# SysCV/LiDAR_snow_sim

Hardware: AMD Instinct MI355X
Metric: augmented points/s/GPU (64x2048 sweep, 2.5 mm/h); HBM roofline % -- value: rows resident in HBM when the clock starts (device-resident API: augment_batch on CUDA tensors); with H2D of the rows and D2H of the results inside the clock: value_pcie_inclusive (higher is better)
Workload: dtype f64

## Files before the change

### lidar_snow_sim_amd/csrc/sg_common.h

```cpp
#pragma once
#include <stddef.h>
#include <stdint.h>

#define SG_PI 3.141592653589793
#define SG_TWO_PI (2 * SG_PI)
#define SG_RBINS 1230
#define SG_NBINS 2048
#define SG_BIN_MARGIN 1e-6
#define SG_BEAM_MARGIN 1e-9
#define SG_TBL_STRIDE 16
#define SG_BLKREC 8
#define SG_HITS_UNDECIDED 0x40000000
#define SG_MAX_LASERS 256
#define SG_LCAP 63
#define SG_TILE 1024

struct SgEntry {
    double phi;
    double x, y, r;
    double t0, t1;
    double rho;
    uint32_t flags;
    uint32_t src;
};

#define SG_OV_CAP 16
#define SG_OV_STRIDE (2 + 3 * SG_OV_CAP)
#ifndef SG_QSTEPS
#define SG_QSTEPS 16
#define SG_QSTEP_M 8.0
#endif

struct SgTable {
    const SgEntry *entries;
    const uint32_t *bin_start;
    const uint32_t *bin_q;
    uint32_t n_bins;
    uint32_t n_entries;
    double inv_bin_w;
    uint32_t n_flakes;
    uint32_t max_bin;
    const uint32_t *bin_qs;
    uint32_t qs_steps;
    float qs_per_m;
};

struct SgLasers {
    double focal_slope[SG_MAX_LASERS];
    double focal_offset[SG_MAX_LASERS];
    int32_t min_i[SG_MAX_LASERS];
    int32_t max_i[SG_MAX_LASERS];
    int32_t n;
};

#define SG_REC_LABEL_SHIFT 8
#define SG_REC_COPY (1u << 10)
#define SG_REC_HAS_I (1u << 11)
#define SG_REC_SLOT (1u << 31)
#define SG_REC_K_SHIFT 12
#define SG_MAX_CLASSES 4

#if defined(__HIPCC__) || defined(__HIP__)
typedef int2 int2_t;
#else
struct int2_t { int32_t x, y; };
#endif

struct SgBeamArgs {
    const void *rows;
    const int64_t *frame_off;
    int32_t n_frames;
    int64_t n_total;
    int64_t uniform_rows;
    float inv_uniform_rows;
    const int32_t *perm;
    const void *srows;
    const int32_t *frame_unsorted;
    const SgTable *frame_tables;
    const SgLasers *las;
    const double *rgrid;
    double beam_div_deg;
    uint32_t *rec;
    uint32_t *rec_q;
    void *rng;
    int32_t *status;
    int32_t *tier_hint;
    unsigned long long *diff2;
    int32_t exact_math;
    int32_t n_cls;
    int32_t cls_cap[SG_MAX_CLASSES];
    const int32_t *seg_blk;
    const int64_t *seg_start;
    const int32_t *seg_cnt;
    const int32_t *seg_frame;
    const int32_t *seg_n;
    const int32_t *seg_of_blk;
    int64_t grid_blocks;
    int32_t q_chunk;
    int64_t blk_lo, blk_hi;
    const int32_t *chunk_blk;
    int32_t chunk;
    uint32_t *dq;
    int32_t *dq_g;
    uint16_t *dq_sc;
    unsigned long long *qn;
    int2_t *pw_items;
    int32_t *pw_count;
    int2_t *pw_items1;
    int32_t front_max;
    int64_t n_regions_ub;
    int32_t blk_rows;
    int32_t kp_lds_quarters;
    int64_t dq_n;
    int32_t *tier_list;
    int32_t *tier_info;
    int64_t tier_stride;
    int32_t *tier_sparse;
    int32_t *tn, *tbase;
    int32_t cls;
    int32_t work_lo, work_hi;
    int32_t work_hint;
    int32_t *redo_list;
    int32_t *redo_cnt;
    double *tq;
    uint16_t *tq_sc;
    int32_t tq_cap;
    double *ov;
    uint16_t *ov_sc;
    int32_t ov_cap;
    int32_t ov_list;
    double *h_lists;
    int32_t h_cap, h_lanes;
    int32_t *dbg_count;
    double *dbg_rj;
    double *dbg_ratio;
    int32_t dbg_cap;
};

struct SgFov {
    int32_t enabled;
    int32_t reserved_;
    double m[12];
    double p[12];
    double img_h, img_w;
};

#ifdef __cplusplus
extern "C" {
#endif
int sg_launch_expand_rows(const void *xyzi, const uint8_t *ch, void *rows, int64_t n, void *stream);
int sg_launch_sort(const void *rows, int dtype, const int64_t *frame_off, int n_frames, int64_t n_total,
                   int32_t *tile_hist, int32_t *tile_base, uint16_t *rank, uint8_t *ch8, int32_t *perm, int32_t *status,
                   int64_t max_tiles_per_frame, const double *lean_plane, double *lean_part, int32_t *tile_unsorted,
                   int32_t *frame_unsorted, void *srows, int identity_perm ,
                   int phase , void *stream);
int sg_launch_gather_rows(const void *rows, int dtype, const int64_t *frame_off, int n_frames, int64_t n_total, int64_t max_frame,
                          const int32_t *perm, void *srows, int32_t *frame_unsorted, int32_t *status, void *stream);
int sg_launch_beams(const SgBeamArgs *args, int dtype, int lmax, int direct, void *stream);
int sg_launch_power(const SgBeamArgs *args, int dtype, int lmax, void *stream, int plan_only ,
                    void *ev_few , int which );
int sg_launch_tier_gather(const SgBeamArgs *args, void *stream);
int sg_launch_power_list(const SgBeamArgs *args, int dtype, int lmax, void *stream);
int sg_launch_huge(const SgBeamArgs *args, int dtype, void *stream);
int sg_launch_tier_scan(const SgBeamArgs *args, int dtype, int lmax, void *stream);
int sg_launch_rows(const SgBeamArgs *args, int dtype, int lmax, void *stream);
int sg_launch_segments(const int64_t *frame_off, int n_frames, const int32_t *tile_base, int64_t max_tiles, const int32_t *table_ids,
                       int n_las, int n_tables, int block, unsigned long long *tbl_cnt, unsigned long long *tbl_base, int32_t *seg_blk,
                       int64_t *seg_start, int32_t *seg_cnt, int32_t *seg_frame, int32_t *seg_n, int32_t *seg_of_blk,
                       int32_t *chunk_blk, const SgTable *tables, SgTable *resolved , void *stream);
int sg_launch_segments_small(const int64_t *frame_off, int n_frames, const int32_t *tile_base, int64_t max_tiles, const int32_t *table_ids,
                             int n_las, int n_tables, int block, int32_t *seg_blk, int64_t *seg_start, int32_t *seg_cnt, int32_t *seg_frame,
                             int32_t *seg_n, int32_t *seg_of_blk, int32_t *chunk_blk, const SgTable *tables, SgTable *resolved,
                             unsigned long long *zero, int64_t n_zero, void *stream);
int sg_beams_block(int lmax);
int sg_launch_resolve_tables(const SgTable *tables, int n_tables, const int32_t *table_ids, int64_t n, SgTable *out, void *stream);
struct SgPackOut {
    uint32_t *meta;
    void *inten;
    void *mv;
    int64_t *mv_counts;
    int32_t *tile_mv, *tile_mv_base;
};
int sg_launch_compact(const void *rows, const void *srows, const int32_t *frame_unsorted, int dtype, const uint32_t *rec, const uint32_t *rec_q, const void *rng, const double *thr_poly, uint8_t *keep, const int32_t *perm,
                      const int64_t *frame_off, int n_frames, int64_t n_total, int32_t *tile_cnt,
                      int32_t *tile_base, void *out_rows, int32_t *out_src, int64_t *out_counts,
                      int64_t *out_stats, const unsigned long long *diff2, const SgFov *fov, int64_t max_tiles_per_frame,
                      const SgPackOut *pack , unsigned long long *tiles_done , void *stream);
int sg_launch_finish_aligned(const void *rows, const void *srows, const int32_t *frame_unsorted, int dtype, const uint32_t *rec, const uint32_t *rec_q, const void *rng,
                             const double *thr_poly, const int32_t *perm, const int64_t *frame_off, int n_frames, int32_t *tile_cnt, int32_t *tile_base,
                             void *out_rows, uint8_t *out_keep, int64_t *out_counts, int64_t *out_stats, const unsigned long long *diff2, const SgFov *fov,
                             int64_t max_tiles_per_frame, unsigned long long *tiles_done , void *stream);
int sg_launch_crop_count(const void *rows, int dtype, const int64_t *frame_off, int n_frames, uint8_t *keep, int32_t *tile_cnt,
                         int32_t *tile_base, int64_t *out_counts, int64_t *stats_scratch, const SgFov *fov, int64_t max_tiles, void *stream);
int sg_launch_crop_scatter(const void *rows, int dtype, const uint8_t *keep, const double *gate , const int64_t *frame_off, const int64_t *new_off,
                           int n_frames, const int32_t *tile_base, void *out_rows, int32_t *crop_src, int64_t max_tiles, void *stream);
int sg_launch_mask_front(const void *rows, int dtype, const uint8_t *keep_in, const double *weather, const int64_t *frame_off, int n_frames, void *out_rows ,
                         uint8_t *out_keep, int32_t *tile_cnt, int32_t *tile_base, int64_t *counts, int64_t *new_off, void *crows, int32_t *map,
                         int64_t max_tiles, void *stream);
int sg_launch_finish_aligned_masked(const void *crows, const void *srows, const int32_t *frame_unsorted, int dtype, const uint32_t *rec, const uint32_t *rec_q,
                                    const void *rng, const double *thr_poly, const int32_t *perm, const int64_t *c_off, const int64_t *in_off,
                                    const int32_t *map, int n_frames, int32_t *tile_cnt, int32_t *tile_base, void *out_rows, uint8_t *out_keep,
                                    int64_t *out_counts, int64_t *out_stats, const unsigned long long *diff2, const SgFov *fov, int64_t max_tiles_per_frame,
                                    unsigned long long *tiles_done , void *stream);
int sg_launch_fov_mask(const void *rows, int dtype, int64_t n, const uint8_t *keep_in, uint8_t *out_keep, const SgFov *fov, void *stream);
struct SgDrorGrid;
int sg_launch_dror(const void *rows, int dtype, int64_t n, const int64_t *frame_off, int n_frames, const uint8_t *keep_in, const struct SgDrorGrid *g,
                   uint32_t *entry, uint32_t *cell_of, void *sorted, uint8_t *out_keep, int32_t *out_nb, void *stream);
struct SgVoxelGrid;
int sg_launch_voxelize(const void *rows, int dtype, int64_t n, const int64_t *frame_off, int n_frames, const uint8_t *keep_in, const struct SgVoxelGrid *g,
                       unsigned long long *table, uint32_t *slot_of, uint8_t *first, uint32_t *order, int32_t *tile_cnt, int32_t *tile_base, int32_t *fbase,
                       int32_t *m, uint32_t *span, void *out_voxels, int32_t *out_coords, int32_t *out_num_points, int32_t *out_voxel_offsets,
                       int32_t *out_voxel_of, void *stream);
struct SgFpsRange;
int sg_launch_fps(const void *rows, int dtype, int64_t n, const int64_t *frame_off, int n_frames, const uint8_t *keep_in, const struct SgFpsRange *range,
                  int32_t n_samples, int32_t n_features, void *sx, void *sy, void *sz, void *st, int32_t *ssrc, int32_t *out_index, void *out_points,
                  void *out_dist, int32_t *out_usable, void *stream);
int sg_launch_fps_sectors(const void *rows, int dtype, int64_t n, int64_t max_frame, const int64_t *frame_off, int n_frames, const uint8_t *keep_in,
                          const struct SgFpsRange *range, int32_t n_samples, int32_t n_features, int32_t n_sectors, const void *rois, int32_t n_rois,
                          int32_t roi_features, double roi_margin, void *sx, void *sy, void *sz, void *st, int32_t *ssrc, int8_t *sec, void *rec,
                          int32_t *tile, int32_t *seg, int32_t *out_index, void *out_points, void *out_dist, int32_t *out_usable,
                          int32_t *out_offsets, int32_t *out_count, int8_t *out_sector_of, double *out_reach2, void *stream);
struct SgBallGrid;
int sg_launch_ball(const void *rows, int dtype, int64_t n, const int64_t *frame_off, int n_frames, const uint8_t *keep_in, const struct SgFpsRange *range,
                   const struct SgBallGrid *g, int32_t n_centres, const void *centres, int32_t centre_features, int n_radii, const double *radii,
                   const int *n_samples, int32_t n_features, uint32_t *entry, uint32_t *cell_of, void *sx, void *sy, void *sz, int32_t *ssrc,
                   int32_t *out_index, int32_t *out_count, void *out_points, void *stream);
struct SgRangeGeom;
int sg_launch_range(const void *rows, int dtype, int64_t n, const int64_t *frame_off, int n_frames, const uint8_t *keep_in, const int32_t *ring,
                    const struct SgRangeGeom *g, int32_t n_features, unsigned long long *key, void *out_image, int32_t *out_index,
                    int32_t *out_pixel_of, int32_t *out_count, void *stream);
struct SgNnGrid;
int sg_launch_nn(const void *rows, int dtype, int64_t n, const int64_t *frame_off, int n_frames, const uint8_t *keep_in, const struct SgFpsRange *range,
                 const struct SgNnGrid *g, int32_t n_centres, const void *centres, int32_t centre_features, int k, uint32_t *entry, int32_t *box, void *rec,
                 int32_t *out_index, void *out_dist, void *out_weight, void *stream);
struct SgBoxRec;
int sg_launch_box(const void *rows, int dtype, int64_t n, const int64_t *frame_off, int n_frames, const uint8_t *keep_in, int32_t n_boxes,
                  const void *boxes, int32_t box_features, const double *pose_in, struct SgBoxRec *rec, unsigned long long *table, int32_t *out_box_of,
                  int32_t *out_count, void *out_local, double *out_pose, void *stream);
int sg_launch_roipool(const void *rows, int dtype, int64_t n, int64_t max_frame, const int64_t *frame_off, int n_frames, const uint8_t *keep_in,
                      int32_t n_rois, const void *rois, int32_t roi_features, const double *ew, int32_t n_samples, int32_t num_features,
                      const double *pose_in, struct SgBoxRec *rec, unsigned long long *table, int32_t *run_cnt, int32_t *out_index, int32_t *out_count,
                      void *out_points, void *out_local, double *out_pose, void *stream);
int sg_launch_roi_members(const void *rows, int dtype, int64_t n, int64_t max_frame, const int64_t *frame_off, int n_frames, const uint8_t *keep_in,
                          int32_t n_rois, const void *rois, int32_t roi_features, const double *ew, int32_t n_slots, const double *pose_in,
                          struct SgBoxRec *rec, unsigned long long *table, int32_t *run_cnt, int32_t *out_index, int32_t *out_count, double *out_pose,
                          void *stream);
int sg_launch_roiaware(const void *rows, int dtype, int64_t n, int64_t max_frame, const int64_t *frame_off, int n_frames, const uint8_t *keep_in,
                       int32_t n_rois, const void *rois, int32_t roi_features, const double *ew, const int32_t *grid, int32_t max_points, int32_t cap,
                       const float *features, int32_t channels, const double *pose_in, struct SgBoxRec *rec, unsigned long long *table, int32_t *run_cnt,
                       int32_t *list, int32_t *sorted, int32_t *offset, int32_t *out_roi_count, int32_t *out_count, int32_t *out_index, float *out_max,
                       int32_t *out_argmax, float *out_avg, double *out_pose, void *stream);
int sg_launch_iou(int n_frames, int32_t M, const void *boxes_a, int32_t a_features, int32_t B, const void *boxes_b, int32_t b_features, int dtype, int mode,
                  const double *pose_a, const double *pose_b, double *rec, void *out_iou, int32_t *out_best, void *out_best_iou, void *stream);
int sg_launch_nms(int n_frames, int32_t B, const void *boxes, int32_t box_features, const void *scores, int dtype, int mode, double iou_thresh,
                  double score_thresh, int32_t post_max, const double *pose_in, double *rec, int32_t *order, int32_t *n_cand, int32_t *out_index,
                  int32_t *out_count, void *out_boxes, void *out_scores, uint8_t *out_kept, void *stream);
struct SgTargetCfg;
int sg_launch_sample_rois(const struct SgTargetCfg *cfg, int n_frames, int32_t n_rois, const void *rois, int32_t roi_features, const void *overlap,
                          const int32_t *assign, int32_t n_gt, const void *gt, int32_t gt_features, int dtype, uint64_t seed, const uint64_t *d_step,
                          const double *pose_in, int32_t *out_index, void *out_rois, void *out_roi_iou, int32_t *out_gt_index, void *out_gt_of_rois,
                          uint8_t *out_reg_valid, void *out_cls_label, int32_t *out_segments, int32_t *out_class_count, double *out_pose,
                          void *out_gt_local, void *stream);
struct SgAnchorCfg;
int sg_launch_assign_anchors(const struct SgAnchorCfg *cfg, int n_frames, int32_t n_anchors, const void *anchors, int32_t anchor_features,
                             const int32_t *anchor_class, int32_t n_gt, const void *gt, int32_t gt_features, int dtype, void *recs,
                             unsigned long long *top, int32_t *blk, int32_t *out_label, int32_t *out_gt_index, int32_t *out_count,
                             int32_t *out_gt_count, void *out_iou, void *stream);
struct SgCenterCfg;
int sg_launch_assign_centers(const struct SgCenterCfg *cfg, int n_frames, int32_t n_gt, const void *gt, int32_t gt_features, int dtype, void *recs,
                             float *out_heatmap, int32_t *out_gt_index, int32_t *out_ind, uint8_t *out_mask, void *out_offset, int32_t *out_radius,
                             int32_t *out_count, uint8_t *out_state, void *stream);
struct SgPasteGroups;
struct SgPasteFrame;
int sg_launch_paste(const void *rows, int dtype, int64_t n_total, int64_t max_frame, const int64_t *off, int n_frames, const uint8_t *keep, int32_t n_gt,
                    const void *gt, int32_t gt_features, const double *pose_in, const void *bank_points, const int64_t *bank_off, const void *bank_boxes,
                    const double *bank_pose, const int32_t *class_off, const struct SgPasteGroups *groups, const double *ew, uint64_t seed,
                    const uint64_t *d_step, int32_t *table, struct SgPasteFrame *frames, unsigned long long *grid, void *out_rows, uint8_t *out_keep, void *out_gt, int32_t *out_object,
                    int32_t *out_state, int32_t *out_source, int32_t *out_count, double *out_pose, void *stream);
struct SgSceneCfg;
int sg_launch_scene(const void *rows, int dtype, int64_t n_total, int64_t max_frame, const int64_t *off, int n_frames, const uint8_t *keep, int32_t B,
                    const void *gt, int32_t Cb, const double *pose_in, const struct SgSceneCfg *cfg, uint64_t seed, const uint64_t *d_step, const int32_t *box_of,
                    struct SgBoxRec *box_rec, unsigned long long *box_table, int32_t *box_of_own, double *tries, double *rowrec, void *out_rows, uint8_t *out_keep,
                    void *out_gt, double *out_world, int32_t *out_state, int32_t *out_tried, double *out_local, double *out_pose, double *out_tries,
                    void *stream);
#ifdef __cplusplus
}
#endif
```

### lidar_snow_sim_amd/csrc/sg_host.h

```cpp
#pragma once
#include <hip/hip_runtime.h>

#include <algorithm>
#include <array>
#include <cmath>
#include <cstdio>
#include <cstdlib>
#include <cstring>
#include <string>
#include <vector>

#include "../../include/snowgpu.h"
#include "sg_common.h"
#include "sg_prepass.h"
#include "sg_plane.h"
#include "sg_assemble.h"
#include "sg_device_args.h"

#pragma GCC visibility push(hidden)

struct DeviceTable {
    SgEntry *entries = nullptr;
    uint32_t *bin_start = nullptr;
    uint32_t *bin_q = nullptr;
    uint32_t *bin_qs = nullptr;
    SgTable desc{};
};

template <typename T> struct DevBuf {
    T *p = nullptr;
    size_t cap = 0;
    int ensure(size_t n)
    {
        if (n <= cap) return 0;
        if (p) (void)hipFree(p);
        p = nullptr;
        cap = 0;
        size_t want = n + n / 4 + 64;
        hipError_t e = hipMalloc((void **)&p, want * sizeof(T));
        if (e != hipSuccess) return (int)e;
        cap = want;
        return 0;
    }
    void release() { if (p) (void)hipFree(p); p = nullptr; cap = 0; }
};

struct __attribute__((visibility("default"))) snowgpu_ctx {
    int device = 0;
    hipStream_t stream = nullptr;
    hipStream_t aux = nullptr;
    hipStream_t aux2 = nullptr;
    hipStream_t aux3 = nullptr;
    int32_t *tier_hint_h = nullptr, *tier_hint_d = nullptr;
    hipEvent_t ev_fork0 = nullptr, ev_join0 = nullptr;
    hipEvent_t ev_fork = nullptr, ev_join = nullptr;
    hipEvent_t ev_fp = nullptr, ev_join2 = nullptr;
    hipEvent_t ev_few = nullptr;
    hipEvent_t ev_lists = nullptr, ev_join3 = nullptr;
    std::string err;
    std::vector<DeviceTable> tables;
    SgTable *d_tables = nullptr;
    size_t d_tables_cap = 0;
    bool tables_dirty = true;
    uint32_t max_flakes = 0;
    SgLasers h_las{};
    SgLasers *d_las = nullptr;
    double *d_rgrid = nullptr;
    int32_t *d_status = nullptr;
    SgFov fov{};
    int fov_pre = 0;
    DevBuf<uint8_t> rows_crop;
    DevBuf<int32_t> crop_src, crop_out_src;
    DevBuf<int64_t> crop_counts, crop_off, crop_stats;
    DevBuf<uint32_t> dror_entry, dror_cell;
    DevBuf<uint8_t> dror_sorted;
    DevBuf<unsigned long long> vox_table;
    DevBuf<uint32_t> vox_slot, vox_order, vox_span;
    DevBuf<uint8_t> vox_first;
    DevBuf<int32_t> vox_tile_cnt, vox_tile_base, vox_fbase, vox_m;
    DevBuf<uint8_t> fps_x, fps_y, fps_z, fps_t;
    DevBuf<int32_t> fps_src;
    DevBuf<int8_t> fpss_sec;
    DevBuf<double> fpss_roi;
    DevBuf<int32_t> fpss_tile, fpss_seg;
    DevBuf<uint32_t> ball_entry, ball_cell;
    DevBuf<uint8_t> ball_x, ball_y, ball_z;
    DevBuf<int32_t> ball_src;
    DevBuf<unsigned long long> range_key;
    DevBuf<uint32_t> nn_entry;
    DevBuf<int32_t> nn_box;
    DevBuf<uint8_t> nn_rec;
    DevBuf<double> box_rec;
    DevBuf<unsigned long long> box_table;
    DevBuf<double> roi_rec;
    DevBuf<unsigned long long> roi_table;
    DevBuf<int32_t> roi_runs;
    DevBuf<double> rv_rec;
    DevBuf<unsigned long long> rv_table;
    DevBuf<int32_t> rv_runs, rv_list, rv_sorted, rv_offset;
    DevBuf<double> iou_rec;
    DevBuf<int32_t> nms_order, nms_cand;
    DevBuf<double> anchor_rec;
    DevBuf<unsigned long long> anchor_top;
    DevBuf<int32_t> anchor_blk;
    DevBuf<double> center_rec;
    DevBuf<int32_t> paste_runs;
    DevBuf<uint8_t> paste_frames;
    DevBuf<unsigned long long> paste_grid;
    DevBuf<double> scene_rowrec, scene_tries, scene_box_rec;
    DevBuf<unsigned long long> scene_box_table;
    DevBuf<int32_t> scene_box_of;
    DevBuf<int32_t> tile_hist, tile_base, perm, ctile_cnt, ctile_base, table_ids, out_src;
    DevBuf<uint8_t> srows;
    DevBuf<int32_t> tile_unsorted, frame_unsorted;
    DevBuf<unsigned long long> seg_tbl_cnt, seg_tbl_base;
    DevBuf<int32_t> seg_blk, seg_cnt, seg_frame, seg_n, seg_of_blk;
    DevBuf<int64_t> seg_start;
    DevBuf<uint32_t> rec, rec_q;
    DevBuf<uint8_t> rng;
    DevBuf<uint32_t> dq;
    DevBuf<int32_t> dq_g;
    DevBuf<uint16_t> dq_sc;
    DevBuf<unsigned long long> qn;
    DevBuf<int2_t> pw_items;
    DevBuf<double> ov;
    DevBuf<uint16_t> ov_sc;
    DevBuf<int32_t> tier_list, tier_sparse, tbase, redo_list;
    DevBuf<double> tq[SG_MAX_CLASSES];
    DevBuf<uint16_t> tq_sc[SG_MAX_CLASSES];
    DevBuf<double> h_lists;
    int64_t tier_cap_override = 0;
    int first_tier_override = 0;
    int few = 2;
    int heavy_tail = -1;
    int tier_rows = -1;
    hipStream_t lane_stream[3] = {nullptr, nullptr, nullptr};
    int stats_early = -1;
    int prepass_with_few = -1;
    bool serial = false;
    DevBuf<int32_t> chunk_blk;
    DevBuf<uint16_t> rank;
    DevBuf<uint8_t> keep, rows_in, rows_out;
    DevBuf<int64_t> frame_off, out_counts, out_stats;
    DevBuf<double> thr_poly, plane, dbg_rj, dbg_ratio, user_thr, out_thr;
    DevBuf<int32_t> user_perm;
    DevBuf<int32_t> dbg_count;
    DevBuf<SgTable> frame_tables;
    SgPrepassScratch prepass{};
    SgPlaneScratch plane_scr{};
    SgPlaneParams plane_par{SG_PLANE_REFERENCE, 1024, 5, 0, -1.55};
    DevBuf<double> plane_est, wet_plane_est;
    DevBuf<int32_t> plane_info;
    int64_t resident_rows = -1;
    int resident_dtype = -1;
    std::vector<int64_t> resident_off;
    DevBuf<int32_t> stats_hist;
    DevBuf<double> stats_rec;
    DevBuf<uint8_t> snow_rows;
    DevBuf<int32_t> snow_src, wet_flags;
    DevBuf<int64_t> snow_counts, wet_counts;
    DevBuf<double> wet_rows, wet_plane;
    std::vector<hipEvent_t> ev_start, ev_stop;
    int ev_used = 0;
    bool prof = false;
    hipStream_t prof_stream = nullptr;
    int exact_math = 0;
    snowgpu_ctx *root = nullptr;
    std::vector<snowgpu_ctx *> lanes;
    int pipe_lanes = 2;
    char *mail_up_h = nullptr, *mail_dn_h = nullptr;
    size_t mail_up_cap = 0, mail_dn_cap = 0;
    DevBuf<uint8_t> mail_up_d, mail_dn_d;
    hipStream_t s_h2d = nullptr, s_d2h = nullptr;
    std::vector<hipEvent_t> pipe_ev;
    DevBuf<int64_t> pipe_off;
    DevBuf<int32_t> pipe_status;
    int64_t pipe_rows = (int64_t)3 << 19;
    std::vector<double> wet_lines;
    DevBuf<double> d_wet_lines;
    int wet_estimation = 0;
    uint64_t wet_seed = 0;
    DevBuf<double> wet_fit;
    int wet_fit_frames = 0;
    int32_t h_status[8] = {0, -1, 0, 0, 0, 0, 0, 0};
    int result_mode = 0;
    int asm_threads = 0;
    DevBuf<uint32_t> pk_meta;
    DevBuf<uint8_t> pk_int, pk_mv;
    DevBuf<int64_t> pk_mvcnt;
    DevBuf<int32_t> pk_tile_mv, pk_tile_mv_base;
    char *st_pk = nullptr;
    size_t st_pk_cap = 0;
    std::vector<hipEvent_t> pk_ev;
    AsmPool *pool = nullptr;
    double pk_times[4] = {0, 0, 0, 0};
    const uint8_t *in_channels = nullptr;
    DevBuf<uint8_t> rows_c4, rows_ch;
    snowgpu_threshold_fn thr_fn = nullptr;
    void *thr_user = nullptr;
    char *thr_stage = nullptr;
    size_t thr_stage_cap = 0;
    std::vector<hipEvent_t> thr_ev;
};

#define HIPCHK(ctx, call)                                                                         \
    do {                                                                                          \
        hipError_t e__ = (call);                                                                  \
        if (e__ != hipSuccess) {                                                                  \
            (ctx)->err = std::string(#call) + ": " + hipGetErrorString(e__);                      \
            return SNOWGPU_E_HIP;                                                                 \
        }                                                                                         \
    } while (0)

#define ENSURE(ctx, buf, n)                                                                       \
    do {                                                                                          \
        if ((buf).ensure(n)) { (ctx)->err = "hipMalloc failed for " #buf; return SNOWGPU_E_HIP; } \
    } while (0)

static inline int fail(snowgpu_ctx *ctx, int code, const std::string &msg)
{
    if (ctx) ctx->err = msg;
    return code;
}

static inline std::array<hipEvent_t *, 9> lane_events(snowgpu_ctx *c)
{
    return {&c->ev_fork0, &c->ev_join0, &c->ev_fork, &c->ev_join, &c->ev_join2, &c->ev_lists, &c->ev_join3, &c->ev_few, &c->ev_fp};
}

struct HostCall {
    snowgpu_ctx *ctx;
    bool pipe = false;
    bool drained = false;
    hipError_t drain()
    {
        drained = true;
        hipError_t first = hipSuccess;
        auto sync = [&first](hipStream_t s) { if (s) { hipError_t e = hipStreamSynchronize(s); if (first == hipSuccess) first = e; } };
        if (pipe) {
            if (ctx->pool) ctx->pool->wait_idle();
            sync(ctx->s_h2d);
            for (snowgpu_ctx *ln : ctx->lanes) sync(ln->stream);
        }
        sync(ctx->stream);
        if (pipe) sync(ctx->s_d2h);
        return first;
    }
    ~HostCall() { if (!drained) (void)drain(); }
};

struct BatchDev {
    int n_frames;
    int64_t n_total;
    int64_t max_frame;
    int64_t uniform_rows = 0;
    const int64_t *frame_off;
    const void *rows;
    int dtype;
    const int32_t *table_ids;
    double beam_div_deg;
    const double *thr_poly;
    const double *plane;
    double noise_floor;
    const int32_t *perm;
    void *out_rows;
    int32_t *out_src;
    uint8_t *out_keep = nullptr;
    const int32_t *mask_map = nullptr;
    const int64_t *mask_in_off = nullptr;
    const double *weather = nullptr;
    int64_t *out_counts;
    int64_t *out_stats;
    double *out_thr_poly;
    int32_t *status;
    hipStream_t stream;
    int32_t *dbg_count = nullptr;
    double *dbg_rj = nullptr, *dbg_ratio = nullptr;
    int dbg_cap = 0;
    int32_t *perm_out = nullptr;
    bool no_fov = false;
    bool want_perm = false;
    SgPackOut *pack = nullptr;
    bool serial = false;
    bool defer_thr = false;
};

int run_batch(snowgpu_ctx *ctx, BatchDev &b);
int run_compaction(snowgpu_ctx *ctx, BatchDev &b);
int status_to_error(snowgpu_ctx *ctx, const int32_t st[8]);
int node_of_device(int device);
SgFov make_fov(const double *v2c, const double *r0, const double *p2, int img_h, int img_w);
int wet_settings(snowgpu_ctx *ctx, const SgWetScalars &w, int n_frames, bool take_lines, hipStream_t st, SgWetParams *wp);

#pragma GCC visibility pop

struct SgWeatherDraw;
extern "C" int sg_launch_draw_weather(const SgWeatherDraw *p, int n_frames, uint64_t seed, const uint64_t *d_step, const int32_t *d_set_ids,
                                      int32_t *d_table_ids, double *d_weather, void *stream);
extern "C" int sg_launch_weather_flags(const double *d_weather, int n_frames, int32_t *d_flags, void *stream);

extern "C" int sg_table_index(const SgEntry *entries, const uint32_t *start, uint32_t *q, uint32_t *qs , int qs_steps, double qs_step_m, void *stream);
extern "C" int sg_file_table_stage_a(const double *d_xyr, int64_t k, SgEntry *fl, int32_t *b0, int32_t *span, uint32_t *count,
                                     uint32_t *start, uint32_t *fill, int32_t *misc, void *stream);
extern "C" int sg_file_table_stage_b(int64_t k, const SgEntry *fl, const int32_t *b0, const int32_t *span, const uint32_t *start,
                                     uint32_t *fill, SgEntry *tmp, SgEntry *entries, void *stream);
extern "C" int sg_table_dump(const SgEntry *entries, uint32_t n_entries, double *d_out, void *stream);
extern "C" int sg_sample_table(double occupancy, double scale_mm, double R0, uint64_t seed, int64_t n_cand, double *d_xyr,
                               int64_t cap, int64_t *n_rows, void *stream);
```

### lidar_snow_sim_amd/csrc/snowgpu_api.cpp

```cpp
#include <dlfcn.h>

#include "sg_host.h"
#include "sg_table_host.h"
#include "sg_range_index.h"
#include <cmath>

static void range_grid(double *out)
{
    const double stop = 120 + 299792458.0 * 1e-8;
    const int num = SG_RBINS;
    const double step = stop / (num - 1);
    for (int k = 0; k < num; ++k) {
        double v = (double)k * step + 0.0;
        if (k == num - 1) v = stop;
        out[k] = std::rint(v * 100.0) / 100.0;
    }
}

extern "C" const char *snowgpu_version(void) { return "snowgpu 0.1.0 gfx950 (MI355X) hip"; }

extern "C" int snowgpu_range_grid(double *out)
{
    if (!out) return SNOWGPU_E_INVALID;
    range_grid(out);
    return SNOWGPU_OK;
}

extern "C" const char *snowgpu_last_error(const snowgpu_ctx *ctx) { return ctx ? ctx->err.c_str() : "null context"; }

static int init_streams(snowgpu_ctx *ctx)
{
    HIPCHK(ctx, hipStreamCreateWithFlags(&ctx->stream, hipStreamNonBlocking));
    {
        int least = 0, greatest = 0;
        (void)hipDeviceGetStreamPriorityRange(&least, &greatest);
        HIPCHK(ctx, hipStreamCreateWithPriority(&ctx->aux, hipStreamNonBlocking, 0));
        HIPCHK(ctx, hipStreamCreateWithPriority(&ctx->aux2, hipStreamNonBlocking, greatest));
        HIPCHK(ctx, hipStreamCreateWithPriority(&ctx->aux3, hipStreamNonBlocking, 0));
    }
    for (hipEvent_t *ep : lane_events(ctx)) HIPCHK(ctx, hipEventCreateWithFlags(ep, hipEventDisableTiming));
    if (hipHostMalloc((void **)&ctx->tier_hint_h, 64, hipHostMallocMapped) == hipSuccess) {
        std::memset(ctx->tier_hint_h, 0, 64);
        if (hipHostGetDevicePointer((void **)&ctx->tier_hint_d, ctx->tier_hint_h, 0) != hipSuccess) ctx->tier_hint_d = nullptr;
    } else { (void)hipGetLastError(); ctx->tier_hint_h = nullptr; }
    return SNOWGPU_OK;
}

extern "C" int snowgpu_create(int device, snowgpu_ctx **out)
{
    if (!out) return SNOWGPU_E_INVALID;
    *out = nullptr;
    int n = 0;
    if (hipGetDeviceCount(&n) != hipSuccess || device < 0 || device >= n) return SNOWGPU_E_NO_DEVICE;
    snowgpu_ctx *ctx = new snowgpu_ctx();
    ctx->device = device;
    *out = ctx;
    HIPCHK(ctx, hipSetDevice(device));
    { const char *v = std::getenv("SNOWGPU_TIER_CAP"); ctx->tier_cap_override = v ? std::atoll(v) : 0; }
    { const char *v = std::getenv("SNOWGPU_FIRST_TIER"); ctx->first_tier_override = v ? std::atoi(v) : 0; }
    { const char *v = std::getenv("SNOWGPU_FEW"); ctx->few = v ? std::max(0, std::min(3, std::atoi(v))) : 2; }
    { const char *v = std::getenv("SNOWGPU_HEAVY_TAIL"); ctx->heavy_tail = v ? (v[0] == '1' ? 1 : 0) : -1; }
    { const char *v = std::getenv("SNOWGPU_SERIAL"); ctx->serial = v && v[0] == '1'; }
    { const char *v = std::getenv("SNOWGPU_STATS_EARLY"); ctx->stats_early = v ? (v[0] == '1' ? 1 : 0) : -1; }
    { const char *v = std::getenv("SNOWGPU_PREPASS_WITH_FEW"); ctx->prepass_with_few = v ? (v[0] == '1' ? 1 : 0) : -1; }
    { const char *v = std::getenv("SNOWGPU_TIER_ROWS"); ctx->tier_rows = v ? (v[0] == '1' ? 1 : 0) : -1; }
    if (void *h = dlopen("libc10_hip.so", RTLD_NOLOAD | RTLD_LAZY)) {
        dlclose(h);
        ctx->pipe_lanes = 1;
        ctx->pipe_rows = (int64_t)3 << 20;
    }
    { const char *v = std::getenv("SNOWGPU_PIPE_LANES"); if (v) ctx->pipe_lanes = std::min(std::max(std::atoi(v), 1), 4); }
    int rc = init_streams(ctx);
    if (rc) return rc;
    HIPCHK(ctx, hipMalloc((void **)&ctx->d_las, sizeof(SgLasers)));
    HIPCHK(ctx, hipMalloc((void **)&ctx->d_rgrid, sizeof(double) * SG_RBINS));
    HIPCHK(ctx, hipMalloc((void **)&ctx->d_status, sizeof(int32_t) * 8));
    double grid[SG_RBINS];
    range_grid(grid);
    HIPCHK(ctx, hipMemcpy(ctx->d_rgrid, grid, sizeof(grid), hipMemcpyHostToDevice));
    ctx->h_las.n = 0;
    return SNOWGPU_OK;
}

extern "C" void snowgpu_destroy(snowgpu_ctx *ctx)
{
    if (!ctx) return;
    (void)hipSetDevice(ctx->device);
    for (snowgpu_ctx *ln : ctx->lanes) snowgpu_destroy(ln);
    ctx->lanes.clear();
    if (ctx->stream) (void)hipStreamSynchronize(ctx->stream);
    for (hipStream_t w : {ctx->s_h2d, ctx->s_d2h, ctx->lane_stream[0], ctx->lane_stream[1], ctx->lane_stream[2]}) if (w) { (void)hipStreamSynchronize(w); (void)hipStreamDestroy(w); }
    if (ctx->tier_hint_h) (void)hipHostFree(ctx->tier_hint_h);
    if (ctx->thr_stage) (void)hipHostFree(ctx->thr_stage);
    for (hipEvent_t e : ctx->thr_ev) (void)hipEventDestroy(e);
    if (ctx->mail_up_h) (void)hipHostFree(ctx->mail_up_h);
    if (ctx->mail_dn_h) (void)hipHostFree(ctx->mail_dn_h);
    ctx->mail_up_d.release(); ctx->mail_dn_d.release(); ctx->d_wet_lines.release(); ctx->wet_fit.release();
    delete ctx->pool; ctx->pool = nullptr;
    if (ctx->st_pk) (void)hipHostFree(ctx->st_pk);
    for (hipEvent_t e : ctx->pk_ev) (void)hipEventDestroy(e);
    ctx->pk_meta.release(); ctx->pk_int.release(); ctx->pk_mv.release(); ctx->pk_mvcnt.release(); ctx->pk_tile_mv.release(); ctx->pk_tile_mv_base.release();
    for (hipEvent_t e : ctx->pipe_ev) (void)hipEventDestroy(e);
    ctx->pipe_off.release(); ctx->pipe_status.release();
    for (auto &t : ctx->tables) {
        if (t.entries) (void)hipFree(t.entries);
        if (t.bin_start) (void)hipFree(t.bin_start);
        if (t.bin_q) (void)hipFree(t.bin_q);
        if (t.bin_qs) (void)hipFree(t.bin_qs);
    }
    if (ctx->d_tables) (void)hipFree(ctx->d_tables);
    if (ctx->d_las) (void)hipFree(ctx->d_las);
    if (ctx->d_rgrid) (void)hipFree(ctx->d_rgrid);
    if (ctx->d_status) (void)hipFree(ctx->d_status);
    ctx->tile_hist.release(); ctx->tile_base.release(); ctx->perm.release(); ctx->srows.release(); ctx->tile_unsorted.release(); ctx->frame_unsorted.release();
    ctx->seg_tbl_cnt.release(); ctx->seg_tbl_base.release(); ctx->seg_blk.release(); ctx->seg_cnt.release(); ctx->seg_frame.release();
    ctx->seg_n.release(); ctx->seg_start.release(); ctx->seg_of_blk.release(); ctx->chunk_blk.release();
    ctx->rec.release(); ctx->rec_q.release(); ctx->rng.release(); ctx->dq.release(); ctx->dq_g.release(); ctx->dq_sc.release(); ctx->qn.release(); ctx->pw_items.release(); ctx->ov.release(); ctx->ov_sc.release();
    ctx->redo_list.release(); ctx->rows_c4.release(); ctx->rows_ch.release();
    ctx->tier_list.release(); ctx->tier_sparse.release(); ctx->tbase.release(); ctx->h_lists.release();
    for (int k = 0; k < SG_MAX_CLASSES; ++k) { ctx->tq[k].release(); ctx->tq_sc[k].release(); }
    ctx->ctile_cnt.release(); ctx->ctile_base.release(); ctx->table_ids.release(); ctx->out_src.release();
    ctx->rank.release(); ctx->keep.release(); ctx->rows_in.release(); ctx->rows_out.release();
    ctx->frame_off.release(); ctx->out_counts.release(); ctx->out_stats.release();
    ctx->thr_poly.release(); ctx->plane.release(); ctx->dbg_rj.release(); ctx->dbg_ratio.release();
    ctx->dbg_count.release(); ctx->frame_tables.release(); ctx->user_thr.release(); ctx->out_thr.release(); ctx->user_perm.release();
    ctx->snow_rows.release(); ctx->snow_src.release(); ctx->wet_flags.release(); ctx->snow_counts.release();
    ctx->wet_counts.release(); ctx->wet_rows.release(); ctx->wet_plane.release();
    ctx->rows_crop.release(); ctx->crop_src.release(); ctx->crop_out_src.release(); ctx->crop_counts.release(); ctx->crop_off.release(); ctx->crop_stats.release();
    ctx->dror_entry.release(); ctx->dror_cell.release(); ctx->dror_sorted.release();
    ctx->vox_table.release(); ctx->vox_slot.release(); ctx->vox_order.release(); ctx->vox_span.release(); ctx->vox_first.release();
    ctx->vox_tile_cnt.release(); ctx->vox_tile_base.release(); ctx->vox_fbase.release(); ctx->vox_m.release();
    ctx->fps_x.release(); ctx->fps_y.release(); ctx->fps_z.release(); ctx->fps_t.release(); ctx->fps_src.release();
    ctx->fpss_sec.release(); ctx->fpss_roi.release(); ctx->fpss_tile.release(); ctx->fpss_seg.release();
    ctx->ball_entry.release(); ctx->ball_cell.release(); ctx->ball_x.release(); ctx->ball_y.release(); ctx->ball_z.release(); ctx->ball_src.release();
    ctx->range_key.release();
    ctx->nn_entry.release(); ctx->nn_box.release(); ctx->nn_rec.release();
    ctx->box_rec.release(); ctx->box_table.release();
    ctx->roi_rec.release(); ctx->roi_table.release(); ctx->roi_runs.release();
    ctx->rv_rec.release(); ctx->rv_table.release(); ctx->rv_runs.release(); ctx->rv_list.release(); ctx->rv_sorted.release(); ctx->rv_offset.release();
    ctx->iou_rec.release(); ctx->nms_order.release(); ctx->nms_cand.release();
    ctx->anchor_rec.release(); ctx->anchor_top.release(); ctx->anchor_blk.release();
    ctx->paste_runs.release(); ctx->paste_frames.release(); ctx->paste_grid.release();
    ctx->scene_rowrec.release(); ctx->scene_tries.release(); ctx->scene_box_rec.release(); ctx->scene_box_table.release(); ctx->scene_box_of.release();
    sg_prepass_release(&ctx->prepass);
    sg_plane_release(&ctx->plane_scr);
    ctx->plane_est.release(); ctx->wet_plane_est.release(); ctx->plane_info.release(); ctx->stats_hist.release(); ctx->stats_rec.release();
    for (auto e : ctx->ev_start) (void)hipEventDestroy(e);
    for (auto e : ctx->ev_stop) (void)hipEventDestroy(e);
    for (hipEvent_t *ep : lane_events(ctx)) if (*ep) (void)hipEventDestroy(*ep);
    for (hipStream_t st : {ctx->aux3, ctx->aux2, ctx->aux, ctx->stream})
        if (st) (void)hipStreamDestroy(st);
    delete ctx;
}

extern "C" int snowgpu_set_lasers(snowgpu_ctx *ctx, int n, const double *focal_slope, const double *focal_offset,
                                  const int32_t *min_intensity, const int32_t *max_intensity)
{
    if (!ctx) return SNOWGPU_E_INVALID;
    if (n <= 0 || n > SG_MAX_LASERS || !focal_slope || !focal_offset || !min_intensity || !max_intensity)
        return fail(ctx, SNOWGPU_E_INVALID, "snowgpu_set_lasers: need 1..256 lasers and four arrays");
    HIPCHK(ctx, hipSetDevice(ctx->device));
    for (int i = 0; i < n; ++i) {
        ctx->h_las.focal_slope[i] = focal_slope[i];
        ctx->h_las.focal_offset[i] = focal_offset[i];
        ctx->h_las.min_i[i] = min_intensity[i];
        ctx->h_las.max_i[i] = max_intensity[i];
    }
    ctx->h_las.n = n;
    HIPCHK(ctx, hipMemcpy(ctx->d_las, &ctx->h_las, sizeof(SgLasers), hipMemcpyHostToDevice));
    return SNOWGPU_OK;
}


static int register_table(snowgpu_ctx *ctx, int table_id, SgEntry *entries, uint32_t *bin_start, uint32_t n_entries, uint32_t k,
                          uint32_t max_bin)
{
    if ((size_t)table_id >= ctx->tables.size()) ctx->tables.resize((size_t)table_id + 1);
    DeviceTable &dt = ctx->tables[(size_t)table_id];
    if (dt.entries || dt.bin_start) (void)hipStreamSynchronize(ctx->stream);
    if (dt.entries) (void)hipFree(dt.entries);
    if (dt.bin_start) (void)hipFree(dt.bin_start);
    if (dt.bin_q) (void)hipFree(dt.bin_q);
    if (dt.bin_qs) (void)hipFree(dt.bin_qs);
    dt.entries = entries; dt.bin_start = bin_start; dt.bin_q = nullptr; dt.bin_qs = nullptr;
    dt.desc = SgTable{};
    ctx->tables_dirty = true;
    uint32_t *q = nullptr, *qs = nullptr;
    int e = (int)hipMalloc((void **)&q, (size_t)SG_NBINS * SG_QSTEPS * sizeof(uint32_t));
    static_assert(SG_QS_FILE_STEPS >= 1 && SG_QS_FILE_STEPS <= 64, "k_table_index files one step per lane of a wave");
    static_assert((float)(1.0 / SG_QS_FILE_STEP_M) * SG_QS_FILE_STEP_M == 1.0, "the step length is a power of two");
    if (!e && SG_QS_FITS(max_bin)) e = (int)hipMalloc((void **)&qs, SG_QS_WORDS_OF(SG_QS_FILE_STEPS, SG_NBINS) * sizeof(uint32_t));
    if (!e) e = sg_table_index(entries, bin_start, q, qs, SG_QS_FILE_STEPS, SG_QS_FILE_STEP_M, ctx->stream);
    if (!e) e = (int)hipStreamSynchronize(ctx->stream);
    if (e) {
        if (q) (void)hipFree(q);
        if (qs) (void)hipFree(qs);
        (void)hipFree(entries); (void)hipFree(bin_start);
        dt.entries = nullptr; dt.bin_start = nullptr;
        return fail(ctx, SNOWGPU_E_HIP, std::string("table index: ") + hipGetErrorString((hipError_t)e));
    }
    dt.bin_q = q; dt.bin_qs = qs;
    dt.desc.entries = entries;
    dt.desc.bin_start = bin_start;
    dt.desc.bin_q = q;
    dt.desc.bin_qs = qs;
    dt.desc.qs_steps = qs ? (uint32_t)SG_QS_FILE_STEPS : 0u;
    dt.desc.qs_per_m = (float)(1.0 / SG_QS_FILE_STEP_M);
    dt.desc.n_bins = (uint32_t)SG_NBINS;
    dt.desc.n_entries = n_entries;
    dt.desc.inv_bin_w = SG_NBINS / SG_TWO_PI;
    dt.desc.n_flakes = k;
    dt.desc.max_bin = max_bin;
    ctx->tables_dirty = true;
    ctx->max_flakes = std::max(ctx->max_flakes, k);
    return SNOWGPU_OK;
}

static int file_table_device(snowgpu_ctx *ctx, int table_id, const double *d_xyr, int64_t k)
{
    hipStream_t st = ctx->stream;
    const size_t nb = SG_NBINS;
    DevBuf<SgEntry> fl, tmp;
    DevBuf<int32_t> b0, span, misc;
    DevBuf<uint32_t> count, start, fill;
    auto cleanup = [&]() { fl.release(); tmp.release(); b0.release(); span.release(); misc.release(); count.release(); start.release(); fill.release(); };
    if (fl.ensure((size_t)std::max<int64_t>(k, 1)) || b0.ensure((size_t)std::max<int64_t>(k, 1)) || span.ensure((size_t)std::max<int64_t>(k, 1)) ||
        misc.ensure(2) || count.ensure(nb + 1) || start.ensure(nb + 1) || fill.ensure(nb + 1)) {
        cleanup();
        return fail(ctx, SNOWGPU_E_HIP, "hipMalloc failed while filing a table");
    }
    int e = sg_file_table_stage_a(d_xyr, k, fl.p, b0.p, span.p, count.p, start.p, fill.p, misc.p, st);
    uint32_t n_entries = 0;
    int32_t h_misc[2] = {0, 0};
    if (!e) e = (int)hipMemcpyAsync(&n_entries, start.p + nb, sizeof(uint32_t), hipMemcpyDeviceToHost, st);
    if (!e) e = (int)hipMemcpyAsync(h_misc, misc.p, sizeof h_misc, hipMemcpyDeviceToHost, st);
    if (!e) e = (int)hipStreamSynchronize(st);
    if (e) { cleanup(); return fail(ctx, SNOWGPU_E_HIP, std::string("table filing: ") + hipGetErrorString((hipError_t)e)); }
    if (h_misc[0] > 0) {
        cleanup();
        char buf[128];
        snprintf(buf, sizeof buf, "table row %d is not a disk clear of the origin", 0x7fffffff - h_misc[0]);
        return fail(ctx, SNOWGPU_E_TABLE, buf);
    }
    if ((size_t)n_entries > (size_t)64 * (size_t)std::max<int64_t>(k, 1) + 4096) {
        cleanup();
        return fail(ctx, SNOWGPU_E_TABLE, "flakes so close to the sensor that they cover most azimuths");
    }
    SgEntry *d_entries = nullptr;
    uint32_t *d_start = nullptr;
    if (tmp.ensure((size_t)n_entries + 1) || hipMalloc((void **)&d_entries, ((size_t)n_entries + 1) * sizeof(SgEntry)) != hipSuccess ||
        hipMalloc((void **)&d_start, (nb + 1) * sizeof(uint32_t)) != hipSuccess) {
        if (d_entries) (void)hipFree(d_entries);
        cleanup();
        return fail(ctx, SNOWGPU_E_HIP, "hipMalloc failed while filing a table");
    }
    e = sg_file_table_stage_b(k, fl.p, b0.p, span.p, start.p, fill.p, tmp.p, d_entries, st);
    if (!e) e = (int)hipMemcpyAsync(d_start, start.p, (nb + 1) * sizeof(uint32_t), hipMemcpyDeviceToDevice, st);
    if (!e) e = (int)hipStreamSynchronize(st);
    cleanup();
    if (e) { (void)hipFree(d_entries); (void)hipFree(d_start); return fail(ctx, SNOWGPU_E_HIP, std::string("table filing: ") + hipGetErrorString((hipError_t)e)); }
    return register_table(ctx, table_id, d_entries, d_start, n_entries, (uint32_t)k, (uint32_t)h_misc[1]);
}

extern "C" int snowgpu_file_table_device(snowgpu_ctx *ctx, int table_id, const double *d_xyr, int64_t n_flakes)
{
    if (!ctx) return SNOWGPU_E_INVALID;
    if (table_id < 0 || table_id > (1 << 20) || n_flakes < 0 || (n_flakes > 0 && !d_xyr))
        return fail(ctx, SNOWGPU_E_INVALID, "snowgpu_file_table_device: bad table id or size");
    HIPCHK(ctx, hipSetDevice(ctx->device));
    return file_table_device(ctx, table_id, d_xyr, n_flakes);
}

extern "C" int snowgpu_debug_table(snowgpu_ctx *ctx, int table_id, double *out, int64_t cap_rows)
{
    if (!ctx || !out) return SNOWGPU_E_INVALID;
    if (table_id < 0 || (size_t)table_id >= ctx->tables.size() || !ctx->tables[(size_t)table_id].entries)
        return fail(ctx, SNOWGPU_E_INVALID, "snowgpu_debug_table: unknown table id");
    const DeviceTable &dt = ctx->tables[(size_t)table_id];
    const size_t k = dt.desc.n_flakes;
    if ((int64_t)k > cap_rows) return fail(ctx, SNOWGPU_E_INVALID, "snowgpu_debug_table: buffer too small");
    HIPCHK(ctx, hipSetDevice(ctx->device));
    DevBuf<double> d;
    if (d.ensure(std::max<size_t>(k * 4, 1))) return fail(ctx, SNOWGPU_E_HIP, "hipMalloc failed");
    int e = sg_table_dump(dt.entries, dt.desc.n_entries, d.p, ctx->stream);
    if (!e && k) e = (int)hipMemcpyAsync(out, d.p, sizeof(double) * 4 * k, hipMemcpyDeviceToHost, ctx->stream);
    if (!e) e = (int)hipStreamSynchronize(ctx->stream);
    d.release();
    if (e) return fail(ctx, SNOWGPU_E_HIP, std::string("table dump: ") + hipGetErrorString((hipError_t)e));
    return SNOWGPU_OK;
}

extern "C" int snowgpu_debug_table_bins(snowgpu_ctx *ctx, int table_id, uint32_t *bin_start, int64_t cap_start, void *entries, int64_t cap_entries,
                                        uint32_t *bin_q, int64_t cap_q, uint32_t *bin_qs, int64_t cap_qs, int64_t *info, double *qs_per_m)
{
    if (!ctx || !bin_start || !entries || !bin_q || !bin_qs || !info || !qs_per_m) return SNOWGPU_E_INVALID;
    if (table_id < 0 || (size_t)table_id >= ctx->tables.size() || !ctx->tables[(size_t)table_id].entries)
        return fail(ctx, SNOWGPU_E_INVALID, "snowgpu_debug_table_bins: unknown table id");
    const DeviceTable &dt = ctx->tables[(size_t)table_id];
    const size_t n_start = (size_t)SG_NBINS + 1, n_rec = (size_t)dt.desc.n_entries + 1, n_q = (size_t)SG_NBINS * SG_QSTEPS;
    const size_t n_qs = dt.bin_qs ? SG_QS_WORDS_OF(dt.desc.qs_steps, SG_NBINS) : 0;
    info[0] = dt.desc.n_flakes; info[1] = dt.desc.n_entries; info[2] = dt.desc.max_bin; info[3] = dt.desc.qs_steps; info[4] = dt.bin_qs ? 1 : 0;
    *qs_per_m = (double)dt.desc.qs_per_m;
    if (cap_start < (int64_t)n_start || cap_entries < (int64_t)n_rec || cap_q < (int64_t)n_q || cap_qs < (int64_t)n_qs)
        return fail(ctx, SNOWGPU_E_INVALID, "snowgpu_debug_table_bins: buffer too small (see info)");
    HIPCHK(ctx, hipSetDevice(ctx->device));
    int e = (int)hipMemcpyAsync(bin_start, dt.bin_start, sizeof(uint32_t) * n_start, hipMemcpyDeviceToHost, ctx->stream);
    if (!e) e = (int)hipMemcpyAsync(entries, dt.entries, sizeof(SgEntry) * n_rec, hipMemcpyDeviceToHost, ctx->stream);
    if (!e) e = (int)hipMemcpyAsync(bin_q, dt.bin_q, sizeof(uint32_t) * n_q, hipMemcpyDeviceToHost, ctx->stream);
    if (!e && n_qs) e = (int)hipMemcpyAsync(bin_qs, dt.bin_qs, sizeof(uint32_t) * n_qs, hipMemcpyDeviceToHost, ctx->stream);
    const int es = (int)hipStreamSynchronize(ctx->stream);
    if (!e) e = es;
    if (e) return fail(ctx, SNOWGPU_E_HIP, std::string("table bins: ") + hipGetErrorString((hipError_t)e));
    return SNOWGPU_OK;
}

extern "C" int snowgpu_upload_table(snowgpu_ctx *ctx, int table_id, const double *xyr, int64_t k)
{
    if (!ctx) return SNOWGPU_E_INVALID;
    if (table_id < 0 || table_id > (1 << 20) || k < 0 || (k > 0 && !xyr))
        return fail(ctx, SNOWGPU_E_INVALID, "snowgpu_upload_table: bad table id or size");
    HIPCHK(ctx, hipSetDevice(ctx->device));
    const int nb = SG_NBINS;
    std::vector<SgEntry> entries;
    std::vector<uint32_t> start;
    uint32_t max_bin = 0;
    int64_t bad_row = -1;
    const int frc = sg_file_table_host(xyr, k, entries, start, max_bin, &bad_row);
    if (frc == 1) {
        char buf[160];
        snprintf(buf, sizeof buf, "snowgpu_upload_table: row %lld (%g, %g, %g) is not a disk clear of the origin",
                 (long long)bad_row, xyr[3 * bad_row], xyr[3 * bad_row + 1], xyr[3 * bad_row + 2]);
        return fail(ctx, SNOWGPU_E_TABLE, buf);
    }
    if (frc == 2) return fail(ctx, SNOWGPU_E_TABLE, "snowgpu_upload_table: flakes so close to the sensor that they cover most azimuths");
    const size_t n_entries = start[(size_t)nb];
    SgEntry *d_entries = nullptr;
    uint32_t *d_start = nullptr;
    HIPCHK(ctx, hipMalloc((void **)&d_entries, (n_entries + 1) * sizeof(SgEntry)));
    if (hipMalloc((void **)&d_start, ((size_t)nb + 1) * sizeof(uint32_t)) != hipSuccess) { (void)hipFree(d_entries); return fail(ctx, SNOWGPU_E_HIP, "hipMalloc failed for bin offsets"); }
    HIPCHK(ctx, hipMemcpy(d_entries, entries.data(), (n_entries + 1) * sizeof(SgEntry), hipMemcpyHostToDevice));
    HIPCHK(ctx, hipMemcpy(d_start, start.data(), ((size_t)nb + 1) * sizeof(uint32_t), hipMemcpyHostToDevice));
    return register_table(ctx, table_id, d_entries, d_start, (uint32_t)n_entries, (uint32_t)k, max_bin);
}

extern "C" int snowgpu_free_table(snowgpu_ctx *ctx, int table_id)
{
    if (!ctx) return SNOWGPU_E_INVALID;
    if (table_id < 0 || (size_t)table_id >= ctx->tables.size()) return fail(ctx, SNOWGPU_E_INVALID, "snowgpu_free_table: unknown table id");
    HIPCHK(ctx, hipSetDevice(ctx->device));
    DeviceTable &dt = ctx->tables[(size_t)table_id];
    if (dt.entries || dt.bin_start) HIPCHK(ctx, hipStreamSynchronize(ctx->stream));
    if (dt.entries) { (void)hipFree(dt.entries); dt.entries = nullptr; }
    if (dt.bin_start) { (void)hipFree(dt.bin_start); dt.bin_start = nullptr; }
    if (dt.bin_q) { (void)hipFree(dt.bin_q); dt.bin_q = nullptr; }
    if (dt.bin_qs) { (void)hipFree(dt.bin_qs); dt.bin_qs = nullptr; }
    dt.desc = SgTable{};
    ctx->tables_dirty = true;
    return SNOWGPU_OK;
}

extern "C" int snowgpu_table_count(const snowgpu_ctx *ctx)
{
    if (!ctx) return 0;
    int n = 0;
    for (auto &t : ctx->tables) n += t.entries != nullptr;
    return n;
}

extern "C" int snowgpu_status_error(snowgpu_ctx *ctx, const int32_t *status8)
{
    if (!ctx || !status8) return SNOWGPU_E_INVALID;
    return status_to_error(ctx, status8);
}

extern "C" int snowgpu_sample_table(snowgpu_ctx *ctx, int table_id, double occupancy_ratio, double diameter_scale_mm, double r_0,
                                    uint64_t seed, double *xyr_out, int64_t cap, int64_t *n_out)
{
    if (!ctx) return SNOWGPU_E_INVALID;
    if (!(occupancy_ratio > 0) || !(occupancy_ratio < 0.05) || !(diameter_scale_mm > 0) || !(r_0 > 0.05) || !(r_0 <= 500.0) || !n_out)
        return fail(ctx, SNOWGPU_E_INVALID, "snowgpu_sample_table: need 0 < occupancy < 0.05, scale > 0, 0.05 < R0 <= 500 m");
    HIPCHK(ctx, hipSetDevice(ctx->device));
    const double target = occupancy_ratio * SG_PI * r_0 * r_0;
    const double s_m = diameter_scale_mm / 1000.0;
    const double mean_area = SG_PI * s_m * s_m / 3.0;
    int64_t n_cand = (int64_t)(1.3 * target / mean_area) + 4096;
    int64_t rows = 0;
    DevBuf<double> d_xyr;
    for (int attempt = 0;; ++attempt) {
        if (n_cand > ((int64_t)1 << 27)) return fail(ctx, SNOWGPU_E_INVALID, "snowgpu_sample_table: table would exceed 2^27 candidates");
        if (d_xyr.ensure((size_t)n_cand * 3)) return fail(ctx, SNOWGPU_E_HIP, "hipMalloc failed for the sampled table");
        int rc = sg_sample_table(occupancy_ratio, diameter_scale_mm, r_0, seed, n_cand, d_xyr.p, n_cand, &rows, ctx->stream);
        if (rc == -2 && attempt < 4) { d_xyr.release(); n_cand *= 2; continue; }
        if (rc != 0) {
            d_xyr.release();
            if (rc > 0) return fail(ctx, SNOWGPU_E_HIP, std::string("sampler: ") + hipGetErrorString((hipError_t)rc));
            return fail(ctx, SNOWGPU_E_TABLE, rc == -3 ? "sampler: a dart overlaps more than 4 earlier darts (occupancy too high for this sampler)"
                                                       : "sampler: acceptance did not settle / target area not reached");
        }
        break;
    }
    *n_out = rows;
    int rc = SNOWGPU_OK;
    if (xyr_out) {
        if (cap < rows) rc = fail(ctx, SNOWGPU_E_INVALID, "snowgpu_sample_table: output buffer too small (see *n_out)");
        else if (rows && hipMemcpy(xyr_out, d_xyr.p, sizeof(double) * 3 * (size_t)rows, hipMemcpyDeviceToHost) != hipSuccess)
            rc = fail(ctx, SNOWGPU_E_HIP, "sampler copy failed");
    }
    if (rc == SNOWGPU_OK && table_id >= 0) rc = file_table_device(ctx, table_id, d_xyr.p, rows);
    d_xyr.release();
    return rc;
}

extern "C" int snowgpu_last_status(snowgpu_ctx *ctx, int32_t *out8)
{
    if (!ctx || !out8) return SNOWGPU_E_INVALID;
    std::memcpy(out8, ctx->h_status, sizeof(int32_t) * 8);
    return SNOWGPU_OK;
}

extern "C" int snowgpu_device_numa_node(int device)
{
    int n = 0;
    if (hipGetDeviceCount(&n) != hipSuccess || device < 0 || device >= n) return -1;
    return node_of_device(device);
}

extern "C" int snowgpu_set_result_transfer(snowgpu_ctx *ctx, int mode, int threads)
{
    if (!ctx) return SNOWGPU_E_INVALID;
    if ((mode != 0 && mode != 1) || threads < 0 || threads > 256) return fail(ctx, SNOWGPU_E_INVALID, "snowgpu_set_result_transfer: mode 0 or 1, 0 <= threads <= 256");
    if (mode == 1) {
        if (ctx->pool && threads != ctx->asm_threads) { delete ctx->pool; ctx->pool = nullptr; }
        ctx->asm_threads = threads;
    }
    ctx->result_mode = mode;
    return SNOWGPU_OK;
}

extern "C" int snowgpu_debug_transfer_times(snowgpu_ctx *ctx, double *out4)
{
    if (!ctx || !out4) return SNOWGPU_E_INVALID;
    for (int i = 0; i < 3; ++i) out4[i] = ctx->pk_times[i];
    out4[3] = ctx->pool ? (double)ctx->pool->threads.size() : 0.0;
    return SNOWGPU_OK;
}

extern "C" int snowgpu_set_pipeline(snowgpu_ctx *ctx, int64_t chunk_rows)
{
    if (!ctx || chunk_rows < 0) return SNOWGPU_E_INVALID;
    ctx->pipe_rows = chunk_rows;
    return SNOWGPU_OK;
}

extern "C" int snowgpu_set_wet_lines(snowgpu_ctx *ctx, int n_frames, const double *lines)
{
    if (!ctx) return SNOWGPU_E_INVALID;
    if (n_frames <= 0 || !lines) { ctx->wet_lines.clear(); return SNOWGPU_OK; }
    ctx->wet_lines.assign(lines, lines + (size_t)n_frames * 4);
    return SNOWGPU_OK;
}

extern "C" int snowgpu_set_wet_estimation(snowgpu_ctx *ctx, int method, uint64_t seed)
{
    if (!ctx) return SNOWGPU_E_INVALID;
    if (method != 0 && method != 1) return fail(ctx, SNOWGPU_E_INVALID, "snowgpu_set_wet_estimation: method 0 (linear) or 1 (poly)");
    ctx->wet_estimation = method;
    ctx->wet_seed = seed;
    return SNOWGPU_OK;
}

extern "C" int snowgpu_wet_last_fit(snowgpu_ctx *ctx, int n_frames, double *out)
{
    if (!ctx || !out || n_frames <= 0) return SNOWGPU_E_INVALID;
    if (n_frames != ctx->wet_fit_frames) return fail(ctx, SNOWGPU_E_INVALID, "snowgpu_wet_last_fit: the last wet-ground call had another number of frames");
    HIPCHK(ctx, hipSetDevice(ctx->device));
    HIPCHK(ctx, hipStreamSynchronize(ctx->stream));
    HIPCHK(ctx, hipMemcpy(out, ctx->wet_fit.p, sizeof(double) * 8 * (size_t)n_frames, hipMemcpyDeviceToHost));
    return SNOWGPU_OK;
}

extern "C" int snowgpu_debug_ransac_polyfit(snowgpu_ctx *ctx, int m, const double *x, const double *y, uint64_t seed, uint64_t frame, double *out4)
{
    if (!ctx || !x || !y || !out4) return SNOWGPU_E_INVALID;
    if (m < 3 || m > 50) return fail(ctx, SNOWGPU_E_INVALID, "snowgpu_debug_ransac_polyfit: 3 <= m <= 50");
    HIPCHK(ctx, hipSetDevice(ctx->device));
    DevBuf<double> d;
    if (d.ensure(2 * 50 + 4)) return fail(ctx, SNOWGPU_E_HIP, "hipMalloc failed");
    int rc = SNOWGPU_OK;
    hipStream_t st = ctx->stream;
    hipError_t e = hipMemcpyAsync(d.p, x, sizeof(double) * (size_t)m, hipMemcpyHostToDevice, st);
    if (e == hipSuccess) e = hipMemcpyAsync(d.p + 50, y, sizeof(double) * (size_t)m, hipMemcpyHostToDevice, st);
    if (e == hipSuccess) e = (hipError_t)sg_debug_ransac_quad(d.p, d.p + 50, m, seed, frame, d.p + 100, st);
    if (e == hipSuccess) e = hipMemcpyAsync(out4, d.p + 100, sizeof(double) * 4, hipMemcpyDeviceToHost, st);
    if (e == hipSuccess) e = hipStreamSynchronize(st);
    if (e != hipSuccess) rc = fail(ctx, SNOWGPU_E_HIP, std::string("ransac tap: ") + hipGetErrorString(e));
    d.release();
    return rc;
}

extern "C" int snowgpu_set_exact_math(snowgpu_ctx *ctx, int on)
{
    if (!ctx) return SNOWGPU_E_INVALID;
    ctx->exact_math = on ? 1 : 0;
    return SNOWGPU_OK;
}

extern "C" int snowgpu_set_serial(snowgpu_ctx *ctx, int on)
{
    if (!ctx) return SNOWGPU_E_INVALID;
    ctx->serial = on != 0;
    return SNOWGPU_OK;
}

extern "C" int snowgpu_lane_stream(snowgpu_ctx *ctx, int level, void **stream)
{
    if (!ctx || !stream || level < 0 || level > 2) return SNOWGPU_E_INVALID;
    *stream = nullptr;
    HIPCHK(ctx, hipSetDevice(ctx->device));
    if (!ctx->lane_stream[level]) {
        int least = 0, greatest = 0;
        (void)hipDeviceGetStreamPriorityRange(&least, &greatest);
        const int prio = level == 0 ? greatest : level == 2 ? least : (least + greatest) / 2;
        HIPCHK(ctx, hipStreamCreateWithPriority(&ctx->lane_stream[level], hipStreamNonBlocking, prio));
    }
    *stream = (void *)ctx->lane_stream[level];
    return SNOWGPU_OK;
}

extern "C" int snowgpu_host_alloc(snowgpu_ctx *ctx, size_t bytes, void **ptr)
{
    if (!ctx || !ptr) return SNOWGPU_E_INVALID;
    *ptr = nullptr;
    HIPCHK(ctx, hipSetDevice(ctx->device));
    HIPCHK(ctx, hipHostMalloc(ptr, std::max<size_t>(bytes, 8), hipHostMallocPortable));
    return SNOWGPU_OK;
}

extern "C" int snowgpu_host_free(snowgpu_ctx *ctx, void *ptr)
{
    (void)ctx;
    if (!ptr) return SNOWGPU_OK;
    return hipHostFree(ptr) == hipSuccess ? SNOWGPU_OK : SNOWGPU_E_HIP;
}

extern "C" int snowgpu_profile_begin(snowgpu_ctx *ctx, int max_launches)
{
    if (!ctx || max_launches <= 0) return SNOWGPU_E_INVALID;
    HIPCHK(ctx, hipSetDevice(ctx->device));
    while ((int)ctx->ev_start.size() < max_launches) {
        hipEvent_t a, b;
        HIPCHK(ctx, hipEventCreate(&a));
        HIPCHK(ctx, hipEventCreate(&b));
        ctx->ev_start.push_back(a);
        ctx->ev_stop.push_back(b);
    }
    ctx->ev_used = 0;
    ctx->prof = true;
    return SNOWGPU_OK;
}

extern "C" int snowgpu_profile_end(snowgpu_ctx *ctx, double *beam_kernel_ms, int *n_launches)
{
    if (!ctx || !beam_kernel_ms || !n_launches) return SNOWGPU_E_INVALID;
    HIPCHK(ctx, hipSetDevice(ctx->device));
    ctx->prof = false;
    double sum = 0.0;
    if (ctx->ev_used > 0) HIPCHK(ctx, hipEventSynchronize(ctx->ev_stop[(size_t)ctx->ev_used - 1]));
    for (int i = 0; i < ctx->ev_used; ++i) {
        float ms = 0.f;
        HIPCHK(ctx, hipEventElapsedTime(&ms, ctx->ev_start[(size_t)i], ctx->ev_stop[(size_t)i]));
        sum += ms;
    }
    *beam_kernel_ms = sum;
    *n_launches = ctx->ev_used;
    ctx->ev_used = 0;
    return SNOWGPU_OK;
}

extern "C" int snowgpu_set_fov_precrop(snowgpu_ctx *ctx, int on)
{
    if (!ctx) return SNOWGPU_E_INVALID;
    ctx->fov_pre = on ? 1 : 0;
    return SNOWGPU_OK;
}

SgFov make_fov(const double *v2c, const double *r0, const double *p2, int img_h, int img_w)
{
    SgFov f{};
    f.enabled = 1;
    for (int i = 0; i < 4; ++i)
        for (int j = 0; j < 3; ++j) {
            double acc = 0.0;
            for (int k = 0; k < 3; ++k) acc = acc + v2c[4 * k + i] * r0[3 * j + k];
            f.m[3 * i + j] = acc;
        }
    for (int i = 0; i < 12; ++i) f.p[i] = p2[i];
    f.img_h = img_h; f.img_w = img_w;
    return f;
}

extern "C" int snowgpu_set_fov(snowgpu_ctx *ctx, int enabled, const double *v2c, const double *r0, const double *p2, int img_h, int img_w)
{
    if (!ctx) return SNOWGPU_E_INVALID;
    if (!enabled) { ctx->fov.enabled = 0; return SNOWGPU_OK; }
    if (!v2c || !r0 || !p2 || img_h <= 0 || img_w <= 0) return fail(ctx, SNOWGPU_E_INVALID, "snowgpu_set_fov: need V2C, R0, P2 and an image size");
    ctx->fov = make_fov(v2c, r0, p2, img_h, img_w);
    return SNOWGPU_OK;
}

extern "C" int snowgpu_set_plane_method(snowgpu_ctx *ctx, int method, uint64_t seed, int max_trials, int min_rows, double standard_height)
{
    if (!ctx) return SNOWGPU_E_INVALID;
    if (method < SG_PLANE_REFERENCE || method > SG_PLANE_RANSAC || max_trials < 0 || max_trials > (1 << 16) || min_rows < 0)
        return fail(ctx, SNOWGPU_E_INVALID, "snowgpu_set_plane_method: method 0 (reference), 1 (least squares) or 2 (ransac); 0 <= trials <= 65536");
    ctx->plane_par.method = method;
    ctx->plane_par.seed = seed;
    ctx->plane_par.trials = max_trials > 0 ? max_trials : 1024;
    ctx->plane_par.min_rows = min_rows;
    ctx->plane_par.std_height = standard_height;
    return SNOWGPU_OK;
}

extern "C" int snowgpu_set_threshold_callback(snowgpu_ctx *ctx, snowgpu_threshold_fn fn, void *user)
{
    if (!ctx) return SNOWGPU_E_INVALID;
    ctx->thr_fn = fn; ctx->thr_user = fn ? user : nullptr;
    return SNOWGPU_OK;
}
```

### lidar_snow_sim_amd/csrc/snowgpu_batch.cpp

```cpp
#include "sg_host.h"
#include "sg_launch.h"
#include "sg_queue.h"

static int sync_tables(snowgpu_ctx *ctx)
{
    if (!ctx->tables_dirty) return SNOWGPU_OK;
    const size_t n = std::max<size_t>(ctx->tables.size(), 1);
    if (n > ctx->d_tables_cap) {
        if (ctx->d_tables) { (void)hipStreamSynchronize(ctx->stream); (void)hipFree(ctx->d_tables); }
        HIPCHK(ctx, hipMalloc((void **)&ctx->d_tables, n * sizeof(SgTable)));
        ctx->d_tables_cap = n;
    }
    std::vector<SgTable> h(n);
    for (size_t i = 0; i < ctx->tables.size(); ++i) h[i] = ctx->tables[i].desc;
    HIPCHK(ctx, hipMemcpy(ctx->d_tables, h.data(), n * sizeof(SgTable), hipMemcpyHostToDevice));
    ctx->tables_dirty = false;
    return SNOWGPU_OK;
}

static void choose_tiers(const snowgpu_ctx *ctx, double beam_div_deg, int tiers[4], int *n_tiers)
{
    const double expect = (double)ctx->max_flakes * (beam_div_deg * (SG_PI / 180.0)) / SG_TWO_PI;
    int first = expect <= 24.0 ? 4 : (expect <= 48.0 ? 8 : (expect <= 96.0 ? 16 : SG_LCAP));
    if (ctx->first_tier_override == 4 || ctx->first_tier_override == 8 || ctx->first_tier_override == 16 ||
        ctx->first_tier_override == SG_LCAP)
        first = ctx->first_tier_override;
    int n = 0;
    for (int c : {4, 8, 16, SG_LCAP})
        if (c >= first) tiers[n++] = c;
    *n_tiers = n;
}

static int64_t tier_queue_cap(const snowgpu_ctx *ctx, int lmax, int64_t n)
{
    if (ctx->tier_cap_override > 0) return std::min<int64_t>(ctx->tier_cap_override, std::max<int64_t>(n, 1));
    const int64_t slot_bytes = (int64_t)sizeof(double) * (3 * (int64_t)lmax + 2) + 2;
    if (std::max<int64_t>(n, 1) * slot_bytes <= ((int64_t)1 << 30)) return std::max<int64_t>(n, 1);
    const int64_t div = lmax <= 8 ? 4 : (lmax <= 16 ? 16 : 64);
    return std::min<int64_t>(std::max<int64_t>(n, 1), std::max<int64_t>(n / div, 4096));
}

static int launch_compaction(snowgpu_ctx *ctx, BatchDev &b, const int32_t *perm, const double *thr, size_t regions, int64_t max_tiles);

int run_batch(snowgpu_ctx *ctx, BatchDev &b)
{
    snowgpu_ctx *R = ctx->root ? ctx->root : ctx;
    if (R->h_las.n <= 0) return fail(ctx, SNOWGPU_E_INVALID, "snowgpu_set_lasers has not been called");
    if (b.beam_div_deg <= 0 || b.beam_div_deg >= 45.0)
        return fail(ctx, SNOWGPU_E_INVALID, "beam divergence must be in (0, 45) degrees");
    int rc = sync_tables(R);
    if (rc) { if (R != ctx) ctx->err = R->err; return rc; }
    const int64_t max_tiles = sg_tiles(b.max_frame);
    const size_t n = (size_t)b.n_total;
    const size_t esz = b.dtype == 0 ? 4 : 8;
    hipStream_t st = b.stream;
    const bool serial = R->serial || b.serial;
    hipStream_t s_aux = serial ? st : ctx->aux, s_aux2 = serial ? st : ctx->aux2, s_aux3 = serial ? st : ctx->aux3;
    HIPCHK(ctx, hipMemsetAsync(b.status, 0, sizeof(int32_t) * 8, st));
    if (n == 0) {
        HIPCHK(ctx, hipMemsetAsync(b.status + 1, 0xff, sizeof(int32_t), st));
        HIPCHK(ctx, hipMemsetAsync(b.out_counts, 0, sizeof(int64_t) * (size_t)b.n_frames, st));
        HIPCHK(ctx, hipMemsetAsync(b.out_stats, 0, sizeof(int64_t) * 3 * (size_t)b.n_frames, st));
        if (b.pack) HIPCHK(ctx, hipMemsetAsync(b.pack->mv_counts, 0, sizeof(int64_t) * (size_t)b.n_frames, st));
        return SNOWGPU_OK;
    }
    const double *thr = b.thr_poly;
    bool pre_forked = false;
    const bool fuse_stats = !b.thr_poly && !b.defer_thr && !b.perm && (b.plane != nullptr || R->plane_par.method == SG_PLANE_REFERENCE);
    const double *early_plane = b.plane;
    double *lean_part = nullptr;
    if (fuse_stats) {
        if (!early_plane) {
            ENSURE(ctx, ctx->plane_est, (size_t)b.n_frames * 4);
            ENSURE(ctx, ctx->plane_info, (size_t)b.n_frames * 4);
            int pe = sg_plane_run(&ctx->plane_scr, &R->plane_par, b.rows, b.dtype, b.frame_off, nullptr, b.n_frames, b.n_total, b.max_frame,
                                  ctx->plane_est.p, ctx->plane_info.p, st);
            if (pe) return fail(ctx, SNOWGPU_E_HIP, std::string("plane estimate: ") + (pe > 0 ? hipGetErrorString((hipError_t)pe) : "allocation"));
            early_plane = ctx->plane_est.p;
        }
        lean_part = sg_prepass_reserve_tiles(&ctx->prepass, b.n_frames, b.max_frame);
        if (!lean_part) return fail(ctx, SNOWGPU_E_HIP, "prepass: allocation");
    }
    bool hist_early = false;
    const bool stats_early = fuse_stats && !serial && early_plane == b.plane && (R->stats_early < 0 ? b.n_frames > 16 : R->stats_early == 1);
    auto launch_prepass = [&]() -> int {
        HIPCHK(ctx, hipEventRecord(ctx->ev_fork0, st));
        HIPCHK(ctx, hipStreamWaitEvent(s_aux2, ctx->ev_fork0, 0));
        const double *pl = fuse_stats ? early_plane : b.plane;
        if (!pl) {
            ENSURE(ctx, ctx->plane_est, (size_t)b.n_frames * 4);
            ENSURE(ctx, ctx->plane_info, (size_t)b.n_frames * 4);
            int pe = sg_plane_run(&ctx->plane_scr, &R->plane_par, b.rows, b.dtype, b.frame_off, nullptr, b.n_frames, b.n_total, b.max_frame,
                                  ctx->plane_est.p, ctx->plane_info.p, s_aux2);
            if (pe) return fail(ctx, SNOWGPU_E_HIP, std::string("plane estimate: ") + (pe > 0 ? hipGetErrorString((hipError_t)pe) : "allocation"));
            pl = ctx->plane_est.p;
        }
        int e = sg_prepass_run(&ctx->prepass, b.rows, b.dtype, b.frame_off, b.n_frames, b.n_total, b.max_frame, pl,
                               b.noise_floor, ctx->thr_poly.p, b.status, s_aux2, fuse_stats ? 1 : 0, ctx->srows.p, ctx->frame_unsorted.p, hist_early ? 1 : 0, b.weather);
        if (e) return fail(ctx, SNOWGPU_E_HIP, std::string("prepass: ") + (e > 0 ? hipGetErrorString((hipError_t)e) : "allocation"));
        if (b.out_thr_poly)
            HIPCHK(ctx, hipMemcpyAsync(b.out_thr_poly, ctx->thr_poly.p, sizeof(double) * 3 * (size_t)b.n_frames, hipMemcpyDeviceToDevice, s_aux2));
        HIPCHK(ctx, hipEventRecord(ctx->ev_join0, s_aux2));
        pre_forked = true;
        return SNOWGPU_OK;
    };
    if (!thr && b.defer_thr) {
    } else if (!thr) {
        ENSURE(ctx, ctx->thr_poly, (size_t)b.n_frames * 3);
        thr = ctx->thr_poly.p;
        if (!serial) {
            HIPCHK(ctx, hipEventRecord(ctx->ev_fork0, st));
            HIPCHK(ctx, hipStreamWaitEvent(s_aux2, ctx->ev_fork0, 0));
            int he = sg_prepass_clear_hist(&ctx->prepass, b.n_frames, s_aux2);
            if (he) return fail(ctx, SNOWGPU_E_HIP, std::string("prepass: ") + (he > 0 ? hipGetErrorString((hipError_t)he) : "allocation"));
            hist_early = true;
            if (fuse_stats && stats_early) {
                int se = sg_prepass_stats_early(&ctx->prepass, b.rows, b.dtype, b.frame_off, b.n_frames, b.max_frame, early_plane, s_aux2);
                if (se) return fail(ctx, SNOWGPU_E_HIP, std::string("prepass statistics: ") + (se > 0 ? hipGetErrorString((hipError_t)se) : "allocation"));
            }
        }
    } else if (b.out_thr_poly) {
        HIPCHK(ctx, hipMemcpyAsync(b.out_thr_poly, thr, sizeof(double) * 3 * (size_t)b.n_frames, hipMemcpyDeviceToDevice, st));
    }
    const int32_t *perm = b.perm;
    ENSURE(ctx, ctx->srows, n * 5 * esz);
    ENSURE(ctx, ctx->frame_unsorted, (size_t)b.n_frames);
    if (!perm) {
        ENSURE(ctx, ctx->tile_hist, (size_t)b.n_frames * (size_t)max_tiles * 256);
        ENSURE(ctx, ctx->tile_base, (size_t)b.n_frames * (size_t)max_tiles * 256);
        ENSURE(ctx, ctx->tile_unsorted, (size_t)b.n_frames * (size_t)max_tiles);
        ENSURE(ctx, ctx->rank, n);
        ENSURE(ctx, ctx->perm, n);
        ENSURE(ctx, ctx->keep, n);
        int e = sg_launch_sort(b.rows, b.dtype, b.frame_off, b.n_frames, b.n_total, ctx->tile_hist.p, ctx->tile_base.p,
                               ctx->rank.p, ctx->keep.p, ctx->perm.p, b.status, max_tiles, (fuse_stats && !stats_early) ? early_plane : nullptr, (fuse_stats && !stats_early) ? lean_part : nullptr,
                               ctx->tile_unsorted.p, ctx->frame_unsorted.p, ctx->srows.p, b.want_perm ? 1 : 0, 1, st);
        if (e) return fail(ctx, SNOWGPU_E_HIP, std::string("sort launch: ") + hipGetErrorString((hipError_t)e));
        perm = ctx->perm.p;
    } else {
        int e = sg_launch_gather_rows(b.rows, b.dtype, b.frame_off, b.n_frames, b.n_total, b.max_frame, perm, ctx->srows.p, ctx->frame_unsorted.p, b.status, st);
        if (e) return fail(ctx, SNOWGPU_E_HIP, std::string("gather launch: ") + hipGetErrorString((hipError_t)e));
    }
    b.perm_out = const_cast<int32_t *>(perm);
    const int64_t n_ft = (int64_t)b.n_frames * R->h_las.n;
    ENSURE(ctx, ctx->frame_tables, (size_t)n_ft);
    int tiers[4], n_tiers = 0;
    choose_tiers(R, b.beam_div_deg, tiers, &n_tiers);
    const int first_block = sg_beams_block(tiers[0]);
    const bool use_seg = !b.perm && R->tables.size() <= 65536 && b.n_frames <= (1 << 22)
                         && b.n_total < ((int64_t)1 << 31);
    if (b.mask_map && !use_seg) return fail(ctx, SNOWGPU_E_INVALID, "a masked batch needs the segment order of the pass over all rows: at most 65536 tables and 2^22 frames");
    if (use_seg) {
        const size_t P = (size_t)b.n_frames * 256;
        ENSURE(ctx, ctx->seg_tbl_cnt, (R->tables.size() + 1) * SG_TBL_STRIDE); ENSURE(ctx, ctx->seg_tbl_base, R->tables.size() + 1);
        ENSURE(ctx, ctx->seg_blk, P); ENSURE(ctx, ctx->seg_cnt, P);
        ENSURE(ctx, ctx->seg_frame, P); ENSURE(ctx, ctx->seg_start, P); ENSURE(ctx, ctx->seg_n, 2);
        ENSURE(ctx, ctx->seg_of_blk, ((size_t)((b.n_total + first_block - 1) / first_block) + P) * SG_BLKREC);
        ENSURE(ctx, ctx->chunk_blk, 2);
    }
    const int64_t total_blocks_ub = (b.n_total + first_block - 1) / first_block + (use_seg ? (int64_t)b.n_frames * 256 : 0);
    static_assert(SG_MAX_CLASSES * sizeof(int32_t) == 2 * sizeof(unsigned long long), "a region's tier counters are two 64-bit words");
    const size_t q_chunk = 8 * (size_t)first_block;
    const size_t regions = std::max<size_t>((size_t)b.n_frames * 256, n / q_chunk + 2);
    const size_t zero_words = 3 * regions + 2 * (size_t)b.n_frames + 8;
    ENSURE(ctx, ctx->qn, zero_words);
    ENSURE(ctx, ctx->tbase, SG_MAX_CLASSES * regions);
    bool seg_small = false;
    if (use_seg) {
        const int se = sg_launch_segments_small(b.frame_off, b.n_frames, ctx->tile_base.p, max_tiles, b.table_ids, R->h_las.n, (int)R->tables.size(), first_block,
                                                ctx->seg_blk.p, ctx->seg_start.p, ctx->seg_cnt.p, ctx->seg_frame.p, ctx->seg_n.p, ctx->seg_of_blk.p,
                                                ctx->chunk_blk.p, R->d_tables, ctx->frame_tables.p, ctx->qn.p, (int64_t)zero_words, st);
        if (se > 0) return fail(ctx, SNOWGPU_E_HIP, std::string("segment launch: ") + hipGetErrorString((hipError_t)se));
        seg_small = se == 0;
    }
    if (!seg_small) {
        HIPCHK(ctx, hipEventRecord(ctx->ev_fork, st));
        HIPCHK(ctx, hipStreamWaitEvent(s_aux, ctx->ev_fork, 0));
        int e = 0;
        if (!use_seg) e = sg_launch_resolve_tables(R->d_tables, (int)R->tables.size(), b.table_ids, n_ft, ctx->frame_tables.p, s_aux);
        if (e) return fail(ctx, SNOWGPU_E_HIP, std::string("table resolve launch: ") + hipGetErrorString((hipError_t)e));
        if (use_seg) {
            e = sg_launch_segments(b.frame_off, b.n_frames, ctx->tile_base.p, max_tiles, b.table_ids, R->h_las.n, (int)R->tables.size(), first_block,
                                   ctx->seg_tbl_cnt.p, ctx->seg_tbl_base.p, ctx->seg_blk.p, ctx->seg_start.p, ctx->seg_cnt.p, ctx->seg_frame.p,
                                   ctx->seg_n.p, ctx->seg_of_blk.p, ctx->chunk_blk.p, R->d_tables, ctx->frame_tables.p, s_aux);
            if (e) return fail(ctx, SNOWGPU_E_HIP, std::string("segment launch: ") + hipGetErrorString((hipError_t)e));
        }
        HIPCHK(ctx, hipEventRecord(ctx->ev_join, s_aux));
    }
    if (!b.perm) {
        int e = sg_launch_sort(b.rows, b.dtype, b.frame_off, b.n_frames, b.n_total, ctx->tile_hist.p, ctx->tile_base.p,
                               ctx->rank.p, ctx->keep.p, ctx->perm.p, b.status, max_tiles, nullptr, nullptr,
                               ctx->tile_unsorted.p, ctx->frame_unsorted.p, ctx->srows.p, b.want_perm ? 1 : 0, 2, st);
        if (e) return fail(ctx, SNOWGPU_E_HIP, std::string("sort launch: ") + hipGetErrorString((hipError_t)e));
    }
    ENSURE(ctx, ctx->rec, n);
    ENSURE(ctx, ctx->rec_q, n);
    ENSURE(ctx, ctx->rng, n * esz);
    ENSURE(ctx, ctx->keep, n);
    ENSURE(ctx, ctx->tier_list, n * (size_t)n_tiers);
    ENSURE(ctx, ctx->tier_sparse, n * (size_t)n_tiers);
    ENSURE(ctx, ctx->ctile_cnt, (size_t)b.n_frames * (size_t)max_tiles + 1);
    ENSURE(ctx, ctx->ctile_base, (size_t)b.n_frames * (size_t)max_tiles + 1);
    SgBeamArgs a{};
    a.rows = b.rows; a.frame_off = b.frame_off; a.n_frames = b.n_frames; a.n_total = b.n_total; a.perm = perm;
    a.srows = ctx->srows.p; a.frame_unsorted = ctx->frame_unsorted.p;
    a.uniform_rows = (b.uniform_rows > 0 && b.n_total < ((int64_t)1 << 31)) ? b.uniform_rows : 0;
    a.inv_uniform_rows = a.uniform_rows > 0 ? 1.0f / (float)a.uniform_rows : 0.0f;
    a.las = R->d_las; a.frame_tables = ctx->frame_tables.p;
    a.rgrid = R->d_rgrid; a.beam_div_deg = b.beam_div_deg; a.rec = ctx->rec.p; a.rec_q = ctx->rec_q.p;
    a.status = b.status;
    a.rng = ctx->rng.p;
    a.dbg_count = b.dbg_count; a.dbg_rj = b.dbg_rj; a.dbg_ratio = b.dbg_ratio; a.dbg_cap = b.dbg_cap;
    a.exact_math = R->exact_math;
    const int n_cls = n_tiers;
    const bool tier_rows = (R->tier_rows < 0 ? b.n_total <= ((int64_t)1 << 19) : R->tier_rows == 1) && R->tier_cap_override <= 0;
    const int h_lanes = 256;
    const int h_cap = (int)std::min<uint32_t>(std::max<uint32_t>(R->max_flakes, 64u), 8192u);
    a.n_cls = n_cls;
    for (int k = 0; k + 1 < n_cls; ++k) a.cls_cap[k] = tiers[k + 1];
    a.cls_cap[n_cls - 1] = h_cap;
    ENSURE(ctx, ctx->h_lists, (size_t)4 * (size_t)(h_cap + 1) * (size_t)h_lanes);
    a.h_lists = ctx->h_lists.p; a.h_cap = h_cap; a.h_lanes = h_lanes;
    a.tier_list = ctx->tier_list.p; a.tier_stride = b.n_total; a.tier_sparse = ctx->tier_sparse.p;
    if (tier_rows) {
        ENSURE(ctx, ctx->redo_list, n * (size_t)n_tiers);
        a.redo_list = ctx->redo_list.p;
    }
    const bool use_ov = tiers[0] < SG_OV_CAP && n_cls >= 2 && !tier_rows &&
                        R->tier_cap_override <= 0 && n * SG_OV_STRIDE * sizeof(double) <= ((size_t)40 << 30);
    int64_t tq_caps[SG_MAX_CLASSES] = {0, 0, 0, 0};
    for (int k = 0; k + 1 < n_cls && !tier_rows; ++k) {
        if (use_ov && tiers[k + 1] <= SG_OV_CAP) continue;
        tq_caps[k] = tier_queue_cap(R, tiers[k + 1], b.n_total);
        ENSURE(ctx, ctx->tq[k], ((size_t)tq_caps[k] + 64) * (3 * (size_t)tiers[k + 1] + 2));
        ENSURE(ctx, ctx->tq_sc[k], (size_t)tq_caps[k]);
    }
    a.q_chunk = (int32_t)q_chunk;
    {
        const size_t slot_words = (size_t)sg_dq_slot_words(tiers[0], sg_dq_hdr(b.dtype == 0 ? 4 : 8));
        if (n * slot_words * sizeof(uint32_t) > ((size_t)64 << 30))
            return fail(ctx, SNOWGPU_E_INVALID, "batch too large for the dict queue of this table density: split it");
        if (b.n_frames >= (1 << 22)) return fail(ctx, SNOWGPU_E_INVALID, "too many frames in one batch");
        ENSURE(ctx, ctx->dq, (n + 64) * slot_words);
        ENSURE(ctx, ctx->dq_g, n);
        ENSURE(ctx, ctx->dq_sc, n);
        if (!seg_small) HIPCHK(ctx, hipMemsetAsync(ctx->qn.p, 0, sizeof(unsigned long long) * zero_words, st));
        a.tn = (int32_t *)(ctx->qn.p + regions); a.tbase = ctx->tbase.p;
        a.diff2 = ctx->qn.p + 3 * regions;
        int32_t *small = (int32_t *)(ctx->qn.p + 3 * regions + (size_t)b.n_frames);
        a.tier_info = small; a.pw_count = small + 8; a.redo_cnt = small + 12;
        a.dq = ctx->dq.p; a.dq_g = ctx->dq_g.p; a.dq_sc = ctx->dq_sc.p; a.qn = ctx->qn.p; a.dq_n = b.n_total;
        const int lanes = first_block < 64 ? first_block : 64;
        a.n_regions_ub = use_seg ? (int64_t)b.n_frames * 256 : (b.n_total + a.q_chunk - 1) / a.q_chunk;
        a.blk_rows = first_block;
        a.kp_lds_quarters = 2;
        const size_t items_cap = n / (size_t)lanes + 2 * (size_t)a.n_regions_ub + 64;
        ENSURE(ctx, ctx->pw_items, 2 * items_cap);
        a.pw_items = ctx->pw_items.p;
        a.pw_items1 = (R->few > 0 && !b.dbg_count && lanes == 64) ? ctx->pw_items.p + items_cap : nullptr;
        a.front_max = a.pw_items1 ? std::min(R->few, std::min(3, tiers[0])) : 1;
    }
    if (use_ov) {
        ENSURE(ctx, ctx->ov, (n + 256) * SG_OV_STRIDE);
        ENSURE(ctx, ctx->ov_sc, n + 256);
        a.ov = ctx->ov.p; a.ov_sc = ctx->ov_sc.p; a.ov_cap = SG_OV_CAP;
    }
    if (use_seg) {
        a.seg_blk = ctx->seg_blk.p; a.seg_start = ctx->seg_start.p; a.seg_cnt = ctx->seg_cnt.p; a.seg_frame = ctx->seg_frame.p;
        a.seg_n = ctx->seg_n.p; a.seg_of_blk = ctx->seg_of_blk.p; a.chunk_blk = ctx->chunk_blk.p;
    }
    const bool few_first = a.pw_items1 && !serial && b.n_total > ((int64_t)1 << 19);
    bool heavy_tail = false;
    if (few_first && n_cls >= 3 && ctx->tier_hint_d) {
        const volatile int32_t *hint = ctx->tier_hint_h;
        long tail = 0;
        for (int k = 2; k < n_cls && k < SG_MAX_CLASSES; ++k) tail += hint[k];
        heavy_tail = R->heavy_tail < 0 ? (tail >= 4096 && tail * 22 > (long)hint[1]) : R->heavy_tail == 1;
        a.tier_hint = ctx->tier_hint_d;
    }
    if (!seg_small) HIPCHK(ctx, hipStreamWaitEvent(st, ctx->ev_join, 0));
    const bool timed = ctx->prof && ctx->ev_used < (int)ctx->ev_start.size();
    if (timed) { HIPCHK(ctx, hipEventRecord(ctx->ev_start[(size_t)ctx->ev_used], st)); ctx->prof_stream = st; }
    int e = 0;
    {
        const int64_t lin_blocks = (b.n_total + first_block - 1) / first_block;
        if (use_seg) {
            a.chunk = 0;
            a.grid_blocks = total_blocks_ub + b.max_frame / first_block + 2;
        } else {
            a.blk_lo = 0; a.blk_hi = lin_blocks;
            a.grid_blocks = lin_blocks;
        }
        e = sg_launch_beams(&a, b.dtype, tiers[0], 1, st);
        if (!e) e = sg_launch_power(&a, b.dtype, tiers[0], st, 1, nullptr, 3);
        if (!e) {
            HIPCHK(ctx, hipEventRecord(ctx->ev_fp, st));
            HIPCHK(ctx, hipStreamWaitEvent(s_aux, ctx->ev_fp, 0));
            e = sg_launch_power(&a, b.dtype, tiers[0], s_aux, 0, few_first ? ctx->ev_few : nullptr, heavy_tail ? 1 : 3);
        }
        if (!e) {
            const bool pre_with_few = R->prepass_with_few < 0 ? heavy_tail : R->prepass_with_few == 1;
            if (pre_with_few && few_first && !b.thr_poly && !b.defer_thr && !pre_forked) { int prc = launch_prepass(); if (prc) return prc; }
            if (few_first) HIPCHK(ctx, hipStreamWaitEvent(st, ctx->ev_few, 0));
            e = sg_launch_tier_gather(&a, st);
        }
    }
    if (e) return fail(ctx, SNOWGPU_E_HIP, std::string("beam launch: ") + hipGetErrorString((hipError_t)e));
    if (!b.thr_poly && !b.defer_thr && !pre_forked) { int prc = launch_prepass(); if (prc) return prc; }
    const bool side3 = n_cls >= 2;
    const bool tail_main = n_cls >= 3 && !serial && !few_first;
    const bool tail_aux = n_cls >= 3 && !serial && !tail_main;
    if (side3) { HIPCHK(ctx, hipEventRecord(ctx->ev_lists, st)); HIPCHK(ctx, hipStreamWaitEvent(s_aux3, ctx->ev_lists, 0)); }
    if (tail_aux) HIPCHK(ctx, hipStreamWaitEvent(s_aux, ctx->ev_lists, 0));
    if (heavy_tail) {
        e = sg_launch_power(&a, b.dtype, tiers[0], st, 0, nullptr, 2);
    }
    int32_t cls_hint[SG_MAX_CLASSES] = {0, 0, 0, 0};
    if (a.tier_hint && ctx->tier_hint_h) {
        const volatile int32_t *hint = ctx->tier_hint_h;
        const int64_t then_k = hint[SG_MAX_CLASSES];
        if (then_k > 0)
            for (int k = 0; k < SG_MAX_CLASSES; ++k)
                cls_hint[k] = (int32_t)std::min<int64_t>(INT32_MAX / 8, ((int64_t)hint[k] * ((b.n_total >> 10) + 1)) / then_k + 64);
    }
    for (int k = 0; k < n_cls && !e; ++k) {
        a.work_hint = k >= 2 ? cls_hint[k] : 0;
        hipStream_t sk = (k == 0 || (tail_main && k >= 2)) ? st : ((tail_aux && k >= 2) ? s_aux : s_aux3);
        a.seg_blk = nullptr;
        a.cls = k;
        if (k == n_cls - 1) {
            e = sg_launch_huge(&a, b.dtype, sk);
            break;
        }
        const int lmax = tiers[k + 1];
        if (use_ov && lmax <= SG_OV_CAP) {
            a.tq = nullptr; a.tq_sc = nullptr; a.tq_cap = 0; a.ov_list = 1;
            a.work_lo = 0; a.work_hi = (int32_t)std::min<int64_t>(b.n_total, INT32_MAX);
            e = sg_launch_power_list(&a, b.dtype, lmax, sk);
            a.ov_list = 0;
            continue;
        }
        if (tier_rows) {
            a.work_lo = 0; a.work_hi = (int32_t)std::min<int64_t>(b.n_total, INT32_MAX);
            e = sg_launch_rows(&a, b.dtype, lmax, sk);
            continue;
        }
        a.tq = ctx->tq[k].p; a.tq_sc = ctx->tq_sc[k].p; a.tq_cap = (int32_t)tq_caps[k];
        a.work_lo = 0; a.work_hi = (int32_t)tq_caps[k];
        e = sg_launch_tier_scan(&a, b.dtype, lmax, sk);
        if (!e) e = sg_launch_power_list(&a, b.dtype, lmax, sk);
        if (!e && tq_caps[k] < b.n_total) {
            a.work_lo = (int32_t)tq_caps[k]; a.work_hi = (int32_t)std::min<int64_t>(b.n_total, INT32_MAX);
            e = sg_launch_beams(&a, b.dtype, lmax, 0, sk);
        }
    }
    if (e) return fail(ctx, SNOWGPU_E_HIP, std::string("tier launch: ") + hipGetErrorString((hipError_t)e));
    if (side3) { HIPCHK(ctx, hipEventRecord(ctx->ev_join3, s_aux3)); HIPCHK(ctx, hipStreamWaitEvent(st, ctx->ev_join3, 0)); }
    HIPCHK(ctx, hipEventRecord(ctx->ev_join2, s_aux));
    HIPCHK(ctx, hipStreamWaitEvent(st, ctx->ev_join2, 0));
    if (timed) { HIPCHK(ctx, hipEventRecord(ctx->ev_stop[(size_t)ctx->ev_used], st)); ctx->ev_used++; }
    if (pre_forked) HIPCHK(ctx, hipStreamWaitEvent(st, ctx->ev_join0, 0));
    if (b.defer_thr && !b.thr_poly) return SNOWGPU_OK;
    return launch_compaction(ctx, b, perm, thr, regions, max_tiles);
}

static int launch_compaction(snowgpu_ctx *ctx, BatchDev &b, const int32_t *perm, const double *thr, size_t regions, int64_t max_tiles)
{
    snowgpu_ctx *R = ctx->root ? ctx->root : ctx;
    hipStream_t st = b.stream;
    unsigned long long *tiles_done = b.n_total <= ((int64_t)1 << 19) ? ctx->qn.p + 3 * regions + (size_t)b.n_frames + 8 : nullptr;
    if (b.out_keep && b.mask_map) {
        int e = sg_launch_finish_aligned_masked(b.rows, ctx->srows.p, ctx->frame_unsorted.p, b.dtype, ctx->rec.p, ctx->rec_q.p, ctx->rng.p, thr, perm, b.frame_off,
                                                b.mask_in_off, b.mask_map, b.n_frames, ctx->ctile_cnt.p, ctx->ctile_base.p, b.out_rows, b.out_keep, b.out_counts,
                                                b.out_stats, ctx->qn.p + 3 * regions, b.no_fov ? nullptr : &R->fov, max_tiles, tiles_done, st);
        if (e) return fail(ctx, SNOWGPU_E_HIP, std::string("masked aligned finish launch: ") + hipGetErrorString((hipError_t)e));
        return SNOWGPU_OK;
    }
    if (b.out_keep) {
        int e = sg_launch_finish_aligned(b.rows, ctx->srows.p, ctx->frame_unsorted.p, b.dtype, ctx->rec.p, ctx->rec_q.p, ctx->rng.p, thr, perm, b.frame_off, b.n_frames,
                                         ctx->ctile_cnt.p, ctx->ctile_base.p, b.out_rows, b.out_keep, b.out_counts, b.out_stats, ctx->qn.p + 3 * regions,
                                         b.no_fov ? nullptr : &R->fov, max_tiles, tiles_done, st);
        if (e) return fail(ctx, SNOWGPU_E_HIP, std::string("aligned finish launch: ") + hipGetErrorString((hipError_t)e));
        return SNOWGPU_OK;
    }
    if (b.pack) {
        ENSURE(ctx, ctx->pk_tile_mv, (size_t)b.n_frames * (size_t)max_tiles + 1);
        ENSURE(ctx, ctx->pk_tile_mv_base, (size_t)b.n_frames * (size_t)max_tiles + 1);
        b.pack->tile_mv = ctx->pk_tile_mv.p; b.pack->tile_mv_base = ctx->pk_tile_mv_base.p;
    }
    int e = sg_launch_compact(b.rows, ctx->srows.p, ctx->frame_unsorted.p, b.dtype, ctx->rec.p, ctx->rec_q.p, ctx->rng.p, thr, ctx->keep.p, perm, b.frame_off, b.n_frames, b.n_total,
                              ctx->ctile_cnt.p, ctx->ctile_base.p, b.out_rows, b.out_src, b.out_counts, b.out_stats,
                              ctx->qn.p + 3 * regions, b.no_fov ? nullptr : &R->fov, max_tiles, b.pack,
                              tiles_done, st);
    if (e) return fail(ctx, SNOWGPU_E_HIP, std::string("compaction launch: ") + hipGetErrorString((hipError_t)e));
    return SNOWGPU_OK;
}

int run_compaction(snowgpu_ctx *ctx, BatchDev &b)
{
    snowgpu_ctx *R = ctx->root ? ctx->root : ctx;
    if (!b.thr_poly) return fail(ctx, SNOWGPU_E_INVALID, "run_compaction without threshold polynomials");
    if (b.n_total == 0) return SNOWGPU_OK;
    const int64_t max_tiles = sg_tiles(b.max_frame);
    int tiers[4], n_tiers = 0;
    choose_tiers(R, b.beam_div_deg, tiers, &n_tiers);
    const size_t q_chunk = 8 * (size_t)sg_beams_block(tiers[0]);
    const size_t regions = std::max<size_t>((size_t)b.n_frames * 256, (size_t)b.n_total / q_chunk + 2);
    if (b.out_thr_poly)
        HIPCHK(ctx, hipMemcpyAsync(b.out_thr_poly, b.thr_poly, sizeof(double) * 3 * (size_t)b.n_frames, hipMemcpyDeviceToDevice, b.stream));
    return launch_compaction(ctx, b, b.perm ? b.perm : ctx->perm.p, b.thr_poly, regions, max_tiles);
}

int status_to_error(snowgpu_ctx *ctx, const int32_t st[8])
{
    char buf[200];
    switch (st[0]) {
    case 0: return SNOWGPU_OK;
    case SNOWGPU_E_RANGE:
        snprintf(buf, sizeof buf, "index out of bounds for the %d-bin range grid: a simulated point lies at >= ~120 m (sorted row %d)", SG_RBINS, st[1]);
        return fail(ctx, SNOWGPU_E_RANGE, buf);
    case SNOWGPU_E_CHANNELS:
        return fail(ctx, SNOWGPU_E_CHANNELS, "channel column holds values other than integers in [0, 255]; pass an explicit permutation");
    case SNOWGPU_E_OVERFLOW:
        snprintf(buf, sizeof buf, "more than %d flakes intersect one beam (sorted row %d): beyond the global-list tier "
                 "(capacity = the largest uploaded table, at most SNOWGPU_MAX_FLAKES_GLOBAL)",
                 (int)std::min<uint32_t>(std::max<uint32_t>(ctx->max_flakes, 64u), 8192u), st[1]);
        return fail(ctx, SNOWGPU_E_OVERFLOW, buf);
    case SNOWGPU_E_GROUND:
        return fail(ctx, SNOWGPU_E_GROUND, "fewer than 3 ground points in a frame");
    case SNOWGPU_E_INVALID:
        return fail(ctx, SNOWGPU_E_INVALID, "a table id in table_ids was never uploaded");
    default:
        snprintf(buf, sizeof buf, "device status %d", st[0]);
        return fail(ctx, SNOWGPU_E_INVALID, buf);
    }
}
```

### lidar_snow_sim_amd/csrc/snowgpu_sort.hip

```cpp
#include <hip/hip_runtime.h>
#include <algorithm>
#include "sg_common.h"
#include "sg_kutil.h"
#include "sg_lean.h"
#include "sg_launch.h"

template <typename T, bool STATS>
__global__ __launch_bounds__(SG_BLOCK) void k_sort_hist(const T *__restrict__ rows, const int64_t *__restrict__ frame_off,
                                                        int32_t *__restrict__ tile_hist, uint16_t *__restrict__ rank,
                                                        uint8_t *__restrict__ ch8, int32_t *__restrict__ status, int64_t max_tiles, SgLeanTile lean,
                                                        int32_t *__restrict__ tile_unsorted)
{
    const int f = blockIdx.y;
    if (blockIdx.x == 0 && f == 0 && threadIdx.x == 0) status[1] = -1;
    const int64_t base = frame_off[f], n = frame_off[f + 1] - base;
    const int64_t tile0 = (int64_t)blockIdx.x * SG_TILE;
    if (tile0 >= n) return;
    __shared__ volatile int cnt[4][256];
    const int tid = threadIdx.x, w = tid >> 6, lane = tid & 63;
    for (int i = tid; i < 4 * 256; i += SG_BLOCK) ((volatile int *)cnt)[i] = 0;
    __syncthreads();
    int my_bucket[4], my_rank[4];
    [[maybe_unused]] T sx[4], sy[4], sz[4], si[4];
    [[maybe_unused]] bool sv[4];
    int descends = 0;
    T sc[4], scp[4];
#pragma unroll
    for (int q = 0; q < 4; ++q) {
        const int64_t r = tile0 + w * 256 + q * 64 + lane;
        const bool valid = r < n;
        const T *p = rows + (base + (valid ? r : 0)) * 5;
        if constexpr (STATS) { sx[q] = p[0]; sy[q] = p[1]; sz[q] = p[2]; si[q] = p[3]; sv[q] = valid; }
        sc[q] = p[4];
        scp[q] = (valid && lane == 0 && r > 0) ? p[-1] : (T)0;
    }
#pragma unroll
    for (int q = 0; q < 4; ++q) {
        const int64_t r = tile0 + w * 256 + q * 64 + lane;
        const bool valid = r < n;
        int bucket = -1;
        const T c_prev = scp[q];
        if (valid) {
            const T c = sc[q];
            const int ci = (int)c;
            if ((T)ci == c && ci >= 0 && ci < 256) bucket = ci;
            else { atomicCAS(&status[0], 0, 5 ); bucket = 255; }
        }
        {
            int before_b = __shfl_up(bucket, 1);
            if (lane == 0) before_b = r > 0 ? (int)c_prev : bucket;
            if (valid && bucket < before_b) descends = 1;
        }
        my_bucket[q] = bucket;
        my_rank[q] = 0;
        if (valid) ch8[base + r] = (uint8_t)bucket;
        unsigned long long same = __ballot(valid);
#pragma unroll
        for (int bit = 0; bit < 8; ++bit) {
            const bool set = (bucket >> bit) & 1;
            const unsigned long long bb = __ballot(set);
            same &= set ? bb : ~bb;
        }
        if (valid) {
            const int before = cnt[w][bucket];
            my_rank[q] = before + __popcll(same & sg_lanemask_lt());
            if ((same & sg_lanemask_lt()) == 0) cnt[w][bucket] = before + __popcll(same);
        }
    }
    const int any_descends = __syncthreads_or(descends);
    for (int q = 0; q < 4; ++q) {
        const int64_t r = tile0 + w * 256 + q * 64 + lane;
        if (r < n) {
            int off = my_rank[q];
            for (int ww = 0; ww < w; ++ww) off += cnt[ww][my_bucket[q]];
            rank[base + r] = (uint16_t)off;
        }
    }
    int32_t *h = tile_hist + ((int64_t)f * max_tiles + blockIdx.x) * 256;
    h[tid] = cnt[0][tid] + cnt[1][tid] + cnt[2][tid] + cnt[3][tid];
    if (tid == 0) tile_unsorted[(int64_t)f * max_tiles + blockIdx.x] = any_descends ? 1 : 0;
    if constexpr (STATS) {
        __shared__ double sm[58];
        lean_tile_stats<T>(lean, f, blockIdx.x, sx, sy, sz, si, sv, sm);
    }
}

__global__ __launch_bounds__(SG_BLOCK) void k_sort_scan(const int64_t *__restrict__ frame_off,
                                                        const int32_t *__restrict__ tile_hist,
                                                        int32_t *__restrict__ tile_base, int64_t max_tiles,
                                                        const int32_t *__restrict__ tile_unsorted, int32_t *__restrict__ frame_unsorted)
{
    const int f = blockIdx.x, v = threadIdx.x;
    const int64_t n = frame_off[f + 1] - frame_off[f];
    const int64_t tiles = (n + SG_TILE - 1) / SG_TILE;
    const int32_t *h = tile_hist + (int64_t)f * max_tiles * 256;
    int32_t *b = tile_base + (int64_t)f * max_tiles * 256;
    int total = 0, uns = 0;
    for (int64_t t = v; t < tiles; t += SG_BLOCK) uns |= tile_unsorted[(int64_t)f * max_tiles + t];
#pragma unroll 8
    for (int64_t t = 0; t < tiles; ++t) total += h[t * 256 + v];
    __shared__ int s[256];
    s[v] = total;
    uns = __syncthreads_or(uns);
    if (v == 0) frame_unsorted[f] = uns ? 1 : 0;
    for (int d = 1; d < 256; d <<= 1) {
        int add = v >= d ? s[v - d] : 0;
        __syncthreads();
        s[v] += add;
        __syncthreads();
    }
    int run = s[v] - total;
#pragma unroll 8
    for (int64_t t = 0; t < tiles; ++t) { b[t * 256 + v] = run; run += h[t * 256 + v]; }
}

template <typename T>
__global__ __launch_bounds__(SG_BLOCK) void k_sort_scatter(const T *__restrict__ rows, const uint8_t *__restrict__ ch8, const int64_t *__restrict__ frame_off,
                                                           const int32_t *__restrict__ tile_hist, const int32_t *__restrict__ tile_base,
                                                           const uint16_t *__restrict__ rank, int32_t *__restrict__ perm, T *__restrict__ srows,
                                                           const int32_t *__restrict__ frame_unsorted, int identity_perm, int64_t max_tiles)
{
    const int f = blockIdx.y;
    const int64_t base = frame_off[f], n = frame_off[f + 1] - base;
    const int64_t tile0 = (int64_t)blockIdx.x * SG_TILE;
    if (tile0 >= n) return;
    const int tid = threadIdx.x;
    if (!frame_unsorted[f]) {
        if (identity_perm)
            for (int q = 0; q < 4; ++q) { const int64_t r = tile0 + q * SG_BLOCK + tid; if (r < n) perm[base + r] = (int32_t)r; }
        return;
    }
    __shared__ T stage[SG_TILE * 5];
    __shared__ int s_dest[SG_TILE];
    __shared__ uint16_t s_src[SG_TILE];
    __shared__ int s_start[256];
    const int32_t *b = tile_base + ((int64_t)f * max_tiles + blockIdx.x) * 256;
    {
        const int c = tile_hist[((int64_t)f * max_tiles + blockIdx.x) * 256 + tid];
        s_start[tid] = c;
        __syncthreads();
        for (int d = 1; d < 256; d <<= 1) {
            const int add = tid >= d ? s_start[tid - d] : 0;
            __syncthreads();
            s_start[tid] += add;
            __syncthreads();
        }
        const int excl = s_start[tid] - c;
        __syncthreads();
        s_start[tid] = excl;
        __syncthreads();
    }
    const int m = (int)(n - tile0 < SG_TILE ? n - tile0 : SG_TILE);
    for (int q = 0; q < 4; ++q) {
        const int i = q * SG_BLOCK + tid;
        if (i < m) {
            const int64_t r = tile0 + i;
            const int ch = ch8[base + r], rk = rank[base + r];
            const int sp = s_start[ch] + rk;
            const T *p = rows + (base + r) * 5;
            const T v0 = p[0], v1 = p[1], v2 = p[2], v3 = p[3], v4 = p[4];
            T *d = stage + sp * 5;
            d[0] = v0; d[1] = v1; d[2] = v2; d[3] = v3; d[4] = v4;
            s_dest[sp] = b[ch] + rk;
            s_src[sp] = (uint16_t)i;
        }
    }
    __syncthreads();
    for (int idx = tid; idx < m * 5; idx += SG_BLOCK) {
        const int sp = idx / 5, j = idx - sp * 5;
        srows[(base + s_dest[sp]) * 5 + j] = stage[idx];
    }
    for (int sp = tid; sp < m; sp += SG_BLOCK) perm[base + s_dest[sp]] = (int32_t)(tile0 + s_src[sp]);
}

template <typename T>
__global__ __launch_bounds__(SG_BLOCK) void k_gather_rows(const T *__restrict__ rows, const int64_t *__restrict__ frame_off, const int32_t *__restrict__ perm,
                                                          T *__restrict__ srows, int32_t *__restrict__ frame_unsorted, int32_t *__restrict__ status)
{
    const int f = blockIdx.y;
    const int64_t base = frame_off[f], n = frame_off[f + 1] - base;
    if (blockIdx.x == 0 && threadIdx.x == 0) frame_unsorted[f] = 1;
    if (blockIdx.x == 0 && f == 0 && threadIdx.x == 0) status[1] = -1;
    for (int64_t r = (int64_t)blockIdx.x * SG_BLOCK + threadIdx.x; r < n; r += (int64_t)gridDim.x * SG_BLOCK) {
        const T *p = rows + (base + perm[base + r]) * 5;
        T *d = srows + (base + r) * 5;
        d[0] = p[0]; d[1] = p[1]; d[2] = p[2]; d[3] = p[3]; d[4] = p[4];
    }
}

struct SgPair { int64_t start; int rows; int key; };

__device__ __forceinline__ SgPair sg_pair(int p, const int64_t *__restrict__ frame_off, const int32_t *__restrict__ tile_base, int64_t max_tiles,
                                          const int32_t *__restrict__ table_ids, int n_las, int n_tables)
{
    SgPair r;
    const int f = p >> 8, c = p & 255;
    const int64_t n = frame_off[f + 1] - frame_off[f];
    r.start = frame_off[f]; r.rows = 0; r.key = n_tables;
    if (n <= 0) return r;
    const int32_t *b = tile_base + (int64_t)f * max_tiles * 256;
    const int64_t s0 = b[c], s1 = c < 255 ? (int64_t)b[c + 1] : n;
    r.start += s0;
    r.rows = (int)(s1 - s0);
    if (c < n_las) {
        const int id = table_ids[(int64_t)f * n_las + c];
        if (id >= 0 && id < n_tables) r.key = id;
    }
    return r;
}

__global__ __launch_bounds__(256) void k_seg_count(const int64_t *__restrict__ frame_off, int n_frames, const int32_t *__restrict__ tile_base,
                                                   int64_t max_tiles, const int32_t *__restrict__ table_ids, int n_las, int n_tables, int blk,
                                                   unsigned long long *__restrict__ tbl_cnt, const SgTable *__restrict__ tables,
                                                   SgTable *__restrict__ resolved)
{
    const int p = blockIdx.x * 256 + threadIdx.x;
    if (p >= n_frames * 256) return;
    if (resolved && (p & 255) < n_las) {
        const int64_t i = (int64_t)(p >> 8) * n_las + (p & 255);
        const int t = table_ids[i];
        SgTable d{};
        if (t >= 0 && t < n_tables) d = tables[t];
        resolved[i] = d;
    }
    const SgPair r = sg_pair(p, frame_off, tile_base, max_tiles, table_ids, n_las, n_tables);
    if (r.rows > 0) atomicAdd(&tbl_cnt[(size_t)r.key * SG_TBL_STRIDE], (1ull << 32) | (unsigned long long)((r.rows + blk - 1) / blk));
}

__global__ __launch_bounds__(1024) void k_seg_scan(unsigned long long *__restrict__ tbl_cnt, unsigned long long *__restrict__ tbl_base, int n,
                                                   int32_t *__restrict__ seg_n, int32_t *__restrict__ one_chunk_blk)
{
    __shared__ unsigned long long sc[1024];
    const int t = threadIdx.x;
    const int per = (n + 1023) / 1024, b0 = t * per, b1 = b0 + per < n ? b0 + per : n;
    unsigned long long sum = 0;
    for (int k = b0; k < b1; ++k) sum += tbl_cnt[(size_t)k * SG_TBL_STRIDE];
    sc[t] = sum;
    __syncthreads();
    for (int d = 1; d < 1024; d <<= 1) { const unsigned long long add = t >= d ? sc[t - d] : 0; __syncthreads(); sc[t] += add; __syncthreads(); }
    unsigned long long run = sc[t] - sum;
    for (int k = b0; k < b1; ++k) { const unsigned long long c = tbl_cnt[(size_t)k * SG_TBL_STRIDE]; tbl_base[k] = run; run += c; tbl_cnt[(size_t)k * SG_TBL_STRIDE] = 0; }
    if (t == 1023) {
        seg_n[0] = (int32_t)(sc[1023] >> 32); seg_n[1] = (int32_t)(sc[1023] & 0xffffffffull);
        if (one_chunk_blk) { one_chunk_blk[0] = 0; one_chunk_blk[1] = (int32_t)(sc[1023] & 0xffffffffull); }
    }
}

__global__ __launch_bounds__(256) void k_seg_place(const int64_t *__restrict__ frame_off, int n_frames, const int32_t *__restrict__ tile_base,
                                                   int64_t max_tiles, const int32_t *__restrict__ table_ids, int n_las, int n_tables, int blk,
                                                   const unsigned long long *__restrict__ tbl_base, unsigned long long *__restrict__ tbl_cur,
                                                   int64_t *__restrict__ seg_start, int32_t *__restrict__ seg_cnt, int32_t *__restrict__ seg_frame,
                                                   int32_t *__restrict__ seg_blk, int32_t *__restrict__ seg_of_blk)
{
    const int p = blockIdx.x * 256 + threadIdx.x;
    if (p >= n_frames * 256) return;
    const SgPair r = sg_pair(p, frame_off, tile_base, max_tiles, table_ids, n_las, n_tables);
    if (r.rows <= 0) return;
    const int nb = (r.rows + blk - 1) / blk;
    const unsigned long long c = atomicAdd(&tbl_cur[(size_t)r.key * SG_TBL_STRIDE], (1ull << 32) | (unsigned long long)nb), base = tbl_base[r.key];
    const int slot = (int)(base >> 32) + (int)(c >> 32);
    const int b0 = (int)(base & 0xffffffffull) + (int)(c & 0xffffffffull);
    seg_start[slot] = r.start; seg_cnt[slot] = r.rows; seg_frame[slot] = (p >> 8) | ((p & 255) << 22); seg_blk[slot] = b0;
    for (int q = 0; q < nb; ++q) {
        int32_t *br = seg_of_blk + (int64_t)(b0 + q) * SG_BLKREC;
        br[0] = slot; br[1] = (int32_t)r.start; br[2] = r.rows; br[3] = (p >> 8) | ((p & 255) << 22); br[4] = b0;
    }
}

#define SG_SEG_SMALL_TABLES 4096
__global__ __launch_bounds__(1024) void k_seg_small(const int64_t *__restrict__ frame_off, int n_frames, const int32_t *__restrict__ tile_base,
                                                    int64_t max_tiles, const int32_t *__restrict__ table_ids, int n_las, int n_tables, int blk,
                                                    int64_t *__restrict__ seg_start, int32_t *__restrict__ seg_cnt, int32_t *__restrict__ seg_frame,
                                                    int32_t *__restrict__ seg_blk, int32_t *__restrict__ seg_of_blk, int32_t *__restrict__ seg_n,
                                                    int32_t *__restrict__ one_chunk_blk, const SgTable *__restrict__ tables, SgTable *__restrict__ resolved,
                                                    unsigned long long *__restrict__ zero, int64_t n_zero)
{
    __shared__ unsigned long long cnt[SG_SEG_SMALL_TABLES + 1], sc[1024];
    const int t = threadIdx.x, p = t;
    for (int64_t i = t; i < n_zero; i += 1024) zero[i] = 0ull;
    for (int i = t; i <= n_tables; i += 1024) cnt[i] = 0ull;
    __syncthreads();
    const bool mine = p < n_frames * 256;
    SgPair r{};
    int nb = 0;
    if (mine) {
        if ((p & 255) < n_las) {
            const int64_t i = (int64_t)(p >> 8) * n_las + (p & 255);
            const int id = table_ids[i];
            SgTable d{};
            if (id >= 0 && id < n_tables) d = tables[id];
            resolved[i] = d;
        }
        r = sg_pair(p, frame_off, tile_base, max_tiles, table_ids, n_las, n_tables);
        nb = (r.rows + blk - 1) / blk;
        if (r.rows > 0) atomicAdd(&cnt[r.key], (1ull << 32) | (unsigned long long)nb);
    }
    __syncthreads();
    const int n = n_tables + 1, per = (n + 1023) / 1024, b0 = t * per, b1 = b0 + per < n ? b0 + per : n;
    unsigned long long sum = 0;
    for (int k = b0; k < b1; ++k) sum += cnt[k];
    sc[t] = sum;
    __syncthreads();
    for (int d = 1; d < 1024; d <<= 1) { const unsigned long long add = t >= d ? sc[t - d] : 0; __syncthreads(); sc[t] += add; __syncthreads(); }
    unsigned long long run = sc[t] - sum;
    for (int k = b0; k < b1; ++k) { const unsigned long long c = cnt[k]; cnt[k] = run; run += c; }
    if (t == 1023) {
        seg_n[0] = (int32_t)(sc[1023] >> 32); seg_n[1] = (int32_t)(sc[1023] & 0xffffffffull);
        one_chunk_blk[0] = 0; one_chunk_blk[1] = (int32_t)(sc[1023] & 0xffffffffull);
    }
    __syncthreads();
    if (mine && r.rows > 0) {
        const unsigned long long c = atomicAdd(&cnt[r.key], (1ull << 32) | (unsigned long long)nb);
        const int slot = (int)(c >> 32), bb = (int)(c & 0xffffffffull);
        seg_start[slot] = r.start; seg_cnt[slot] = r.rows; seg_frame[slot] = (p >> 8) | ((p & 255) << 22); seg_blk[slot] = bb;
        for (int q = 0; q < nb; ++q) {
            int32_t *br = seg_of_blk + (int64_t)(bb + q) * SG_BLKREC;
            br[0] = slot; br[1] = (int32_t)r.start; br[2] = r.rows; br[3] = (p >> 8) | ((p & 255) << 22); br[4] = bb;
        }
    }
}

__global__ __launch_bounds__(256) void k_expand_rows(const float4 *__restrict__ xyzi, const uint8_t *__restrict__ ch, float *__restrict__ rows, int64_t n)
{
    const int64_t i = (int64_t)blockIdx.x * 256 + threadIdx.x;
    if (i >= n) return;
    const float4 v = xyzi[i];
    float *r = rows + i * 5;
    r[0] = v.x; r[1] = v.y; r[2] = v.z; r[3] = v.w; r[4] = (float)ch[i];
}


__global__ void k_resolve_tables(const SgTable *__restrict__ tables, int n_tables, const int32_t *__restrict__ table_ids,
                                 int64_t n, SgTable *__restrict__ out)
{
    const int64_t i = (int64_t)blockIdx.x * blockDim.x + threadIdx.x;
    if (i >= n) return;
    const int t = table_ids[i];
    SgTable d{};
    if (t >= 0 && t < n_tables) d = tables[t];
    out[i] = d;
}


extern "C" int sg_launch_expand_rows(const void *xyzi, const uint8_t *ch, void *rows, int64_t n, void *stream)
{
    if (n <= 0) return 0;
    hipLaunchKernelGGL(k_expand_rows, dim3((unsigned)((n + 255) / 256)), dim3(256), 0, (hipStream_t)stream, (const float4 *)xyzi, ch, (float *)rows, n);
    SG_CHECK_LAUNCH();
    return 0;
}

extern "C" int sg_launch_resolve_tables(const SgTable *tables, int n_tables, const int32_t *table_ids, int64_t n, SgTable *out,
                                        void *stream)
{
    if (n <= 0) return 0;
    hipLaunchKernelGGL(k_resolve_tables, dim3((unsigned)((n + 255) / 256)), dim3(256), 0, (hipStream_t)stream, tables, n_tables,
                       table_ids, n, out);
    SG_CHECK_LAUNCH();
    return 0;
}

extern "C" int sg_launch_sort(const void *rows, int dtype, const int64_t *frame_off, int n_frames, int64_t n_total,
                              int32_t *tile_hist, int32_t *tile_base, uint16_t *rank, uint8_t *ch8, int32_t *perm, int32_t *status,
                              int64_t max_tiles, const double *lean_plane, double *lean_part, int32_t *tile_unsorted, int32_t *frame_unsorted,
                              void *srows, int identity_perm, int phase , void *stream)
{
    (void)n_total;
    hipStream_t st = (hipStream_t)stream;
    dim3 grid((unsigned)max_tiles, (unsigned)n_frames);
    SgLeanTile lt{};
    lt.plane = lean_plane; lt.delta = 0.5; lt.part = lean_part; lt.max_tiles = max_tiles;
    return sg_by_dtype(dtype, [&](auto t) {
        using T = decltype(t);
        if (phase & 1) {
            if (lean_plane && lean_part) hipLaunchKernelGGL((k_sort_hist<T, true>), grid, dim3(SG_BLOCK), 0, st, (const T *)rows, frame_off, tile_hist, rank, ch8, status, max_tiles, lt, tile_unsorted);
            else hipLaunchKernelGGL((k_sort_hist<T, false>), grid, dim3(SG_BLOCK), 0, st, (const T *)rows, frame_off, tile_hist, rank, ch8, status, max_tiles, lt, tile_unsorted);
            SG_CHECK_LAUNCH();
            hipLaunchKernelGGL(k_sort_scan, dim3(n_frames), dim3(SG_BLOCK), 0, st, frame_off, tile_hist, tile_base, max_tiles, tile_unsorted, frame_unsorted);
            SG_CHECK_LAUNCH();
        }
        if (phase & 2) {
            hipLaunchKernelGGL(k_sort_scatter<T>, grid, dim3(SG_BLOCK), 0, st, (const T *)rows, ch8, frame_off, tile_hist, tile_base, rank, perm, (T *)srows, frame_unsorted, identity_perm, max_tiles);
            SG_CHECK_LAUNCH();
        }
        return 0;
    });
}

extern "C" int sg_launch_gather_rows(const void *rows, int dtype, const int64_t *frame_off, int n_frames, int64_t n_total, int64_t max_frame,
                                     const int32_t *perm, void *srows, int32_t *frame_unsorted, int32_t *status, void *stream)
{
    (void)n_total;
    if (n_frames <= 0) return 0;
    hipStream_t st = (hipStream_t)stream;
    dim3 grid((unsigned)std::max<int64_t>(1, std::min<int64_t>((max_frame + SG_BLOCK - 1) / SG_BLOCK, 256)), (unsigned)n_frames);
    return sg_by_dtype(dtype, [&](auto t) {
        using T = decltype(t);
        hipLaunchKernelGGL(k_gather_rows<T>, grid, dim3(SG_BLOCK), 0, st, (const T *)rows, frame_off, perm, (T *)srows, frame_unsorted, status);
        SG_CHECK_LAUNCH();
        return 0;
    });
}

extern "C" int sg_launch_segments_small(const int64_t *frame_off, int n_frames, const int32_t *tile_base, int64_t max_tiles, const int32_t *table_ids,
                                        int n_las, int n_tables, int block, int32_t *seg_blk, int64_t *seg_start, int32_t *seg_cnt, int32_t *seg_frame,
                                        int32_t *seg_n, int32_t *seg_of_blk, int32_t *chunk_blk, const SgTable *tables, SgTable *resolved,
                                        unsigned long long *zero, int64_t n_zero, void *stream)
{
    if (n_frames * 256 > 1024 || n_tables + 1 > SG_SEG_SMALL_TABLES || n_zero > (1 << 16)) return -1;
    hipLaunchKernelGGL(k_seg_small, dim3(1), dim3(1024), 0, (hipStream_t)stream, frame_off, n_frames, tile_base, max_tiles, table_ids, n_las, n_tables, block,
                       seg_start, seg_cnt, seg_frame, seg_blk, seg_of_blk, seg_n, chunk_blk, tables, resolved, zero, n_zero);
    SG_CHECK_LAUNCH();
    return 0;
}

extern "C" int sg_launch_segments(const int64_t *frame_off, int n_frames, const int32_t *tile_base, int64_t max_tiles, const int32_t *table_ids,
                                  int n_las, int n_tables, int block, unsigned long long *tbl_cnt, unsigned long long *tbl_base, int32_t *seg_blk,
                                  int64_t *seg_start, int32_t *seg_cnt, int32_t *seg_frame, int32_t *seg_n, int32_t *seg_of_blk,
                                  int32_t *chunk_blk, const SgTable *tables, SgTable *resolved, void *stream)
{
    hipStream_t st = (hipStream_t)stream;
    const unsigned grid = (unsigned)n_frames;
    if (hipMemsetAsync(tbl_cnt, 0, sizeof(unsigned long long) * ((size_t)n_tables + 1) * SG_TBL_STRIDE, st) != hipSuccess) return (int)hipGetLastError();
    hipLaunchKernelGGL(k_seg_count, dim3(grid), dim3(256), 0, st, frame_off, n_frames, tile_base, max_tiles, table_ids, n_las, n_tables, block, tbl_cnt,
                       tables, resolved);
    SG_CHECK_LAUNCH();
    hipLaunchKernelGGL(k_seg_scan, dim3(1), dim3(1024), 0, st, tbl_cnt, tbl_base, n_tables + 1, seg_n, chunk_blk);
    SG_CHECK_LAUNCH();
    hipLaunchKernelGGL(k_seg_place, dim3(grid), dim3(256), 0, st, frame_off, n_frames, tile_base, max_tiles, table_ids, n_las, n_tables, block,
                       tbl_base, tbl_cnt, seg_start, seg_cnt, seg_frame, seg_blk, seg_of_blk);
    SG_CHECK_LAUNCH();
    return 0;
}
```

Measured before the change: 10.45 billion.

## Fold segment counting and zeroing into sort scan, coarsen scatter, skip redundant memsets

Moves the per-table segment count and table resolve into the sort scan kernel, which also zeroes the queue counters, removing the separate k_seg_count kernel and a memset. The counter buffer is kept clean across calls, with a separate cursor array reset by the scan, so the memset is skipped on later calls. A device-written hint about whether any frame was unsorted lets the host run segment placement on the side stream only when needed. When frames are expected to be sorted, the scatter kernel processes several tiles per block. The changes add cross-call state and depend on a host-visible hint from the previous call.

```diff
diff --git a/lidar_snow_sim_amd/csrc/sg_common.h b/lidar_snow_sim_amd/csrc/sg_common.h
--- a/lidar_snow_sim_amd/csrc/sg_common.h
+++ b/lidar_snow_sim_amd/csrc/sg_common.h
@@ -9,6 +9,7 @@
 #define SG_BIN_MARGIN 1e-6
 #define SG_BEAM_MARGIN 1e-9
 #define SG_TBL_STRIDE 16
+#define SG_HINT_UNSORTED 8
 #define SG_BLKREC 8
 #define SG_HITS_UNDECIDED 0x40000000
 #define SG_MAX_LASERS 256
@@ -148,12 +149,19 @@
 #ifdef __cplusplus
 extern "C" {
 #endif
+struct SgSortSeg {
+    const int32_t *table_ids; int n_las, n_tables, block;
+    unsigned long long *tbl_cnt;
+    const SgTable *tables; SgTable *resolved;
+    unsigned long long *zero; int64_t n_zero;
+};
 int sg_launch_expand_rows(const void *xyzi, const uint8_t *ch, void *rows, int64_t n, void *stream);
 int sg_launch_sort(const void *rows, int dtype, const int64_t *frame_off, int n_frames, int64_t n_total,
                    int32_t *tile_hist, int32_t *tile_base, uint16_t *rank, uint8_t *ch8, int32_t *perm, int32_t *status,
                    int64_t max_tiles_per_frame, const double *lean_plane, double *lean_part, int32_t *tile_unsorted,
                    int32_t *frame_unsorted, void *srows, int identity_perm ,
-                   int phase , void *stream);
+                   int phase ,
+                   const struct SgSortSeg *seg , int scatter_tiles , void *stream);
 int sg_launch_gather_rows(const void *rows, int dtype, const int64_t *frame_off, int n_frames, int64_t n_total, int64_t max_frame,
                           const int32_t *perm, void *srows, int32_t *frame_unsorted, int32_t *status, void *stream);
 int sg_launch_beams(const SgBeamArgs *args, int dtype, int lmax, int direct, void *stream);
@@ -165,9 +173,10 @@
 int sg_launch_tier_scan(const SgBeamArgs *args, int dtype, int lmax, void *stream);
 int sg_launch_rows(const SgBeamArgs *args, int dtype, int lmax, void *stream);
 int sg_launch_segments(const int64_t *frame_off, int n_frames, const int32_t *tile_base, int64_t max_tiles, const int32_t *table_ids,
-                       int n_las, int n_tables, int block, unsigned long long *tbl_cnt, unsigned long long *tbl_base, int32_t *seg_blk,
-                       int64_t *seg_start, int32_t *seg_cnt, int32_t *seg_frame, int32_t *seg_n, int32_t *seg_of_blk,
-                       int32_t *chunk_blk, const SgTable *tables, SgTable *resolved , void *stream);
+                       int n_las, int n_tables, int block, unsigned long long *tbl_cnt, unsigned long long *tbl_cur, unsigned long long *tbl_base,
+                       int32_t *seg_blk, int64_t *seg_start, int32_t *seg_cnt, int32_t *seg_frame, int32_t *seg_n, int32_t *seg_of_blk,
+                       int32_t *chunk_blk, const int32_t *frame_unsorted, int32_t *hint_unsorted , void *stream);
+int sg_segments_small_fits(int n_frames, int n_tables, int64_t n_zero);
 int sg_launch_segments_small(const int64_t *frame_off, int n_frames, const int32_t *tile_base, int64_t max_tiles, const int32_t *table_ids,
                              int n_las, int n_tables, int block, int32_t *seg_blk, int64_t *seg_start, int32_t *seg_cnt, int32_t *seg_frame,
                              int32_t *seg_n, int32_t *seg_of_blk, int32_t *chunk_blk, const SgTable *tables, SgTable *resolved,
diff --git a/lidar_snow_sim_amd/csrc/sg_host.h b/lidar_snow_sim_amd/csrc/sg_host.h
--- a/lidar_snow_sim_amd/csrc/sg_host.h
+++ b/lidar_snow_sim_amd/csrc/sg_host.h
@@ -113,7 +113,8 @@
     DevBuf<int32_t> tile_hist, tile_base, perm, ctile_cnt, ctile_base, table_ids, out_src;
     DevBuf<uint8_t> srows;
     DevBuf<int32_t> tile_unsorted, frame_unsorted;
-    DevBuf<unsigned long long> seg_tbl_cnt, seg_tbl_base;
+    DevBuf<unsigned long long> seg_tbl_cnt, seg_tbl_cur, seg_tbl_base;
+    bool seg_cnt_clean = false;
     DevBuf<int32_t> seg_blk, seg_cnt, seg_frame, seg_n, seg_of_blk;
     DevBuf<int64_t> seg_start;
     DevBuf<uint32_t> rec, rec_q;
diff --git a/lidar_snow_sim_amd/csrc/snowgpu_api.cpp b/lidar_snow_sim_amd/csrc/snowgpu_api.cpp
--- a/lidar_snow_sim_amd/csrc/snowgpu_api.cpp
+++ b/lidar_snow_sim_amd/csrc/snowgpu_api.cpp
@@ -113,7 +113,7 @@
     if (ctx->d_rgrid) (void)hipFree(ctx->d_rgrid);
     if (ctx->d_status) (void)hipFree(ctx->d_status);
     ctx->tile_hist.release(); ctx->tile_base.release(); ctx->perm.release(); ctx->srows.release(); ctx->tile_unsorted.release(); ctx->frame_unsorted.release();
-    ctx->seg_tbl_cnt.release(); ctx->seg_tbl_base.release(); ctx->seg_blk.release(); ctx->seg_cnt.release(); ctx->seg_frame.release();
+    ctx->seg_tbl_cnt.release(); ctx->seg_tbl_cur.release(); ctx->seg_tbl_base.release(); ctx->seg_blk.release(); ctx->seg_cnt.release(); ctx->seg_frame.release();
     ctx->seg_n.release(); ctx->seg_start.release(); ctx->seg_of_blk.release(); ctx->chunk_blk.release();
     ctx->rec.release(); ctx->rec_q.release(); ctx->rng.release(); ctx->dq.release(); ctx->dq_g.release(); ctx->dq_sc.release(); ctx->qn.release(); ctx->pw_items.release(); ctx->ov.release(); ctx->ov_sc.release();
     ctx->redo_list.release(); ctx->rows_c4.release(); ctx->rows_ch.release();
diff --git a/lidar_snow_sim_amd/csrc/snowgpu_batch.cpp b/lidar_snow_sim_amd/csrc/snowgpu_batch.cpp
--- a/lidar_snow_sim_amd/csrc/snowgpu_batch.cpp
+++ b/lidar_snow_sim_amd/csrc/snowgpu_batch.cpp
@@ -122,6 +122,48 @@
     } else if (b.out_thr_poly) {
         HIPCHK(ctx, hipMemcpyAsync(b.out_thr_poly, thr, sizeof(double) * 3 * (size_t)b.n_frames, hipMemcpyDeviceToDevice, st));
     }
+    const int64_t n_ft = (int64_t)b.n_frames * R->h_las.n;
+    ENSURE(ctx, ctx->frame_tables, (size_t)n_ft);
+    int tiers[4], n_tiers = 0;
+    choose_tiers(R, b.beam_div_deg, tiers, &n_tiers);
+    const int first_block = sg_beams_block(tiers[0]);
+    const bool use_seg = !b.perm && R->tables.size() <= 65536 && b.n_frames <= (1 << 22)
+                         && b.n_total < ((int64_t)1 << 31);
+    if (b.mask_map && !use_seg) return fail(ctx, SNOWGPU_E_INVALID, "a masked batch needs the segment order of the pass over all rows: at most 65536 tables and 2^22 frames");
+    if (use_seg) {
+        const size_t P = (size_t)b.n_frames * 256;
+        const size_t cnt_cap = ctx->seg_tbl_cnt.cap;
+        ENSURE(ctx, ctx->seg_tbl_cnt, (R->tables.size() + 1) * SG_TBL_STRIDE); ENSURE(ctx, ctx->seg_tbl_cur, (R->tables.size() + 1) * SG_TBL_STRIDE);
+        ENSURE(ctx, ctx->seg_tbl_base, R->tables.size() + 1);
+        if (ctx->seg_tbl_cnt.cap != cnt_cap) ctx->seg_cnt_clean = false;
+        ENSURE(ctx, ctx->seg_blk, P); ENSURE(ctx, ctx->seg_cnt, P);
+        ENSURE(ctx, ctx->seg_frame, P); ENSURE(ctx, ctx->seg_start, P); ENSURE(ctx, ctx->seg_n, 2);
+        ENSURE(ctx, ctx->seg_of_blk, ((size_t)((b.n_total + first_block - 1) / first_block) + P) * SG_BLKREC);
+        ENSURE(ctx, ctx->chunk_blk, 2);
+    }
+    const int64_t total_blocks_ub = (b.n_total + first_block - 1) / first_block + (use_seg ? (int64_t)b.n_frames * 256 : 0);
+    static_assert(SG_MAX_CLASSES * sizeof(int32_t) == 2 * sizeof(unsigned long long), "a region's tier counters are two 64-bit words");
+    const size_t q_chunk = 8 * (size_t)first_block;
+    const size_t regions = std::max<size_t>((size_t)b.n_frames * 256, n / q_chunk + 2);
+    const size_t zero_words = 3 * regions + 2 * (size_t)b.n_frames + 8;
+    ENSURE(ctx, ctx->qn, zero_words);
+    ENSURE(ctx, ctx->tbase, SG_MAX_CLASSES * regions);
+    const bool seg_small = use_seg && sg_segments_small_fits(b.n_frames, (int)R->tables.size(), (int64_t)zero_words);
+    const bool seg_chain = use_seg && !seg_small;
+    const bool expect_unsorted = ctx->tier_hint_h ? ((const volatile int32_t *)ctx->tier_hint_h)[SG_HINT_UNSORTED] != 0 : true;
+    const bool seg_aside = seg_chain && expect_unsorted && !serial;
+    SgSortSeg sseg{};
+    bool seg_cnt_filled = false;
+    if (seg_chain) {
+        if (!ctx->seg_cnt_clean) {
+            HIPCHK(ctx, hipMemsetAsync(ctx->seg_tbl_cnt.p, 0, sizeof(unsigned long long) * ctx->seg_tbl_cnt.cap, st));
+            seg_cnt_filled = true;
+        }
+        ctx->seg_cnt_clean = false;
+        sseg.table_ids = b.table_ids; sseg.n_las = R->h_las.n; sseg.n_tables = (int)R->tables.size(); sseg.block = first_block;
+        sseg.tbl_cnt = ctx->seg_tbl_cnt.p; sseg.tables = R->d_tables; sseg.resolved = ctx->frame_tables.p;
+        sseg.zero = ctx->qn.p; sseg.n_zero = (int64_t)zero_words;
+    }
     const int32_t *perm = b.perm;
     ENSURE(ctx, ctx->srows, n * 5 * esz);
     ENSURE(ctx, ctx->frame_unsorted, (size_t)b.n_frames);
@@ -134,7 +176,7 @@
         ENSURE(ctx, ctx->keep, n);
         int e = sg_launch_sort(b.rows, b.dtype, b.frame_off, b.n_frames, b.n_total, ctx->tile_hist.p, ctx->tile_base.p,
                                ctx->rank.p, ctx->keep.p, ctx->perm.p, b.status, max_tiles, (fuse_stats && !stats_early) ? early_plane : nullptr, (fuse_stats && !stats_early) ? lean_part : nullptr,
-                               ctx->tile_unsorted.p, ctx->frame_unsorted.p, ctx->srows.p, b.want_perm ? 1 : 0, 1, st);
+                               ctx->tile_unsorted.p, ctx->frame_unsorted.p, ctx->srows.p, b.want_perm ? 1 : 0, 1, seg_chain ? &sseg : nullptr, 1, st);
         if (e) return fail(ctx, SNOWGPU_E_HIP, std::string("sort launch: ") + hipGetErrorString((hipError_t)e));
         perm = ctx->perm.p;
     } else {
@@ -142,55 +184,36 @@
         if (e) return fail(ctx, SNOWGPU_E_HIP, std::string("gather launch: ") + hipGetErrorString((hipError_t)e));
     }
     b.perm_out = const_cast<int32_t *>(perm);
-    const int64_t n_ft = (int64_t)b.n_frames * R->h_las.n;
-    ENSURE(ctx, ctx->frame_tables, (size_t)n_ft);
-    int tiers[4], n_tiers = 0;
-    choose_tiers(R, b.beam_div_deg, tiers, &n_tiers);
-    const int first_block = sg_beams_block(tiers[0]);
-    const bool use_seg = !b.perm && R->tables.size() <= 65536 && b.n_frames <= (1 << 22)
-                         && b.n_total < ((int64_t)1 << 31);
-    if (b.mask_map && !use_seg) return fail(ctx, SNOWGPU_E_INVALID, "a masked batch needs the segment order of the pass over all rows: at most 65536 tables and 2^22 frames");
-    if (use_seg) {
-        const size_t P = (size_t)b.n_frames * 256;
-        ENSURE(ctx, ctx->seg_tbl_cnt, (R->tables.size() + 1) * SG_TBL_STRIDE); ENSURE(ctx, ctx->seg_tbl_base, R->tables.size() + 1);
-        ENSURE(ctx, ctx->seg_blk, P); ENSURE(ctx, ctx->seg_cnt, P);
-        ENSURE(ctx, ctx->seg_frame, P); ENSURE(ctx, ctx->seg_start, P); ENSURE(ctx, ctx->seg_n, 2);
-        ENSURE(ctx, ctx->seg_of_blk, ((size_t)((b.n_total + first_block - 1) / first_block) + P) * SG_BLKREC);
-        ENSURE(ctx, ctx->chunk_blk, 2);
-    }
-    const int64_t total_blocks_ub = (b.n_total + first_block - 1) / first_block + (use_seg ? (int64_t)b.n_frames * 256 : 0);
-    static_assert(SG_MAX_CLASSES * sizeof(int32_t) == 2 * sizeof(unsigned long long), "a region's tier counters are two 64-bit words");
-    const size_t q_chunk = 8 * (size_t)first_block;
-    const size_t regions = std::max<size_t>((size_t)b.n_frames * 256, n / q_chunk + 2);
-    const size_t zero_words = 3 * regions + 2 * (size_t)b.n_frames + 8;
-    ENSURE(ctx, ctx->qn, zero_words);
-    ENSURE(ctx, ctx->tbase, SG_MAX_CLASSES * regions);
-    bool seg_small = false;
-    if (use_seg) {
+    if (seg_small) {
         const int se = sg_launch_segments_small(b.frame_off, b.n_frames, ctx->tile_base.p, max_tiles, b.table_ids, R->h_las.n, (int)R->tables.size(), first_block,
                                                 ctx->seg_blk.p, ctx->seg_start.p, ctx->seg_cnt.p, ctx->seg_frame.p, ctx->seg_n.p, ctx->seg_of_blk.p,
                                                 ctx->chunk_blk.p, R->d_tables, ctx->frame_tables.p, ctx->qn.p, (int64_t)zero_words, st);
-        if (se > 0) return fail(ctx, SNOWGPU_E_HIP, std::string("segment launch: ") + hipGetErrorString((hipError_t)se));
-        seg_small = se == 0;
-    }
-    if (!seg_small) {
+        if (se) return fail(ctx, SNOWGPU_E_HIP, std::string("segment launch: ") + (se > 0 ? hipGetErrorString((hipError_t)se) : "not a small batch"));
+    } else if (seg_chain) {
+        if (seg_aside) {
+            HIPCHK(ctx, hipEventRecord(ctx->ev_fork, st));
+            HIPCHK(ctx, hipStreamWaitEvent(s_aux, ctx->ev_fork, 0));
+        }
+        const int e = sg_launch_segments(b.frame_off, b.n_frames, ctx->tile_base.p, max_tiles, b.table_ids, R->h_las.n, (int)R->tables.size(), first_block,
+                                         ctx->seg_tbl_cnt.p, ctx->seg_tbl_cur.p, ctx->seg_tbl_base.p, ctx->seg_blk.p, ctx->seg_start.p, ctx->seg_cnt.p,
+                                         ctx->seg_frame.p, ctx->seg_n.p, ctx->seg_of_blk.p, ctx->chunk_blk.p, ctx->frame_unsorted.p,
+                                         ctx->tier_hint_d ? ctx->tier_hint_d + SG_HINT_UNSORTED : nullptr, seg_aside ? s_aux : st);
+        if (e) return fail(ctx, SNOWGPU_E_HIP, std::string("segment launch: ") + hipGetErrorString((hipError_t)e));
+        if (seg_aside) HIPCHK(ctx, hipEventRecord(ctx->ev_join, s_aux));
+        hipStreamCaptureStatus cap = hipStreamCaptureStatusNone;
+        if (seg_cnt_filled && hipStreamIsCapturing(st, &cap) != hipSuccess) { (void)hipGetLastError(); cap = hipStreamCaptureStatusActive; }
+        ctx->seg_cnt_clean = !(seg_cnt_filled && cap != hipStreamCaptureStatusNone);
+    } else {
         HIPCHK(ctx, hipEventRecord(ctx->ev_fork, st));
         HIPCHK(ctx, hipStreamWaitEvent(s_aux, ctx->ev_fork, 0));
-        int e = 0;
-        if (!use_seg) e = sg_launch_resolve_tables(R->d_tables, (int)R->tables.size(), b.table_ids, n_ft, ctx->frame_tables.p, s_aux);
+        const int e = sg_launch_resolve_tables(R->d_tables, (int)R->tables.size(), b.table_ids, n_ft, ctx->frame_tables.p, s_aux);
         if (e) return fail(ctx, SNOWGPU_E_HIP, std::string("table resolve launch: ") + hipGetErrorString((hipError_t)e));
-        if (use_seg) {
-            e = sg_launch_segments(b.frame_off, b.n_frames, ctx->tile_base.p, max_tiles, b.table_ids, R->h_las.n, (int)R->tables.size(), first_block,
-                                   ctx->seg_tbl_cnt.p, ctx->seg_tbl_base.p, ctx->seg_blk.p, ctx->seg_start.p, ctx->seg_cnt.p, ctx->seg_frame.p,
-                                   ctx->seg_n.p, ctx->seg_of_blk.p, ctx->chunk_blk.p, R->d_tables, ctx->frame_tables.p, s_aux);
-            if (e) return fail(ctx, SNOWGPU_E_HIP, std::string("segment launch: ") + hipGetErrorString((hipError_t)e));
-        }
         HIPCHK(ctx, hipEventRecord(ctx->ev_join, s_aux));
     }
     if (!b.perm) {
         int e = sg_launch_sort(b.rows, b.dtype, b.frame_off, b.n_frames, b.n_total, ctx->tile_hist.p, ctx->tile_base.p,
                                ctx->rank.p, ctx->keep.p, ctx->perm.p, b.status, max_tiles, nullptr, nullptr,
-                               ctx->tile_unsorted.p, ctx->frame_unsorted.p, ctx->srows.p, b.want_perm ? 1 : 0, 2, st);
+                               ctx->tile_unsorted.p, ctx->frame_unsorted.p, ctx->srows.p, b.want_perm ? 1 : 0, 2, nullptr, expect_unsorted ? 1 : 8, st);
         if (e) return fail(ctx, SNOWGPU_E_HIP, std::string("sort launch: ") + hipGetErrorString((hipError_t)e));
     }
     ENSURE(ctx, ctx->rec, n);
@@ -244,7 +267,7 @@
         ENSURE(ctx, ctx->dq, (n + 64) * slot_words);
         ENSURE(ctx, ctx->dq_g, n);
         ENSURE(ctx, ctx->dq_sc, n);
-        if (!seg_small) HIPCHK(ctx, hipMemsetAsync(ctx->qn.p, 0, sizeof(unsigned long long) * zero_words, st));
+        if (!use_seg) HIPCHK(ctx, hipMemsetAsync(ctx->qn.p, 0, sizeof(unsigned long long) * zero_words, st));
         a.tn = (int32_t *)(ctx->qn.p + regions); a.tbase = ctx->tbase.p;
         a.diff2 = ctx->qn.p + 3 * regions;
         int32_t *small = (int32_t *)(ctx->qn.p + 3 * regions + (size_t)b.n_frames);
@@ -278,7 +301,7 @@
         heavy_tail = R->heavy_tail < 0 ? (tail >= 4096 && tail * 22 > (long)hint[1]) : R->heavy_tail == 1;
         a.tier_hint = ctx->tier_hint_d;
     }
-    if (!seg_small) HIPCHK(ctx, hipStreamWaitEvent(st, ctx->ev_join, 0));
+    if (!use_seg || seg_aside) HIPCHK(ctx, hipStreamWaitEvent(st, ctx->ev_join, 0));
     const bool timed = ctx->prof && ctx->ev_used < (int)ctx->ev_start.size();
     if (timed) { HIPCHK(ctx, hipEventRecord(ctx->ev_start[(size_t)ctx->ev_used], st)); ctx->prof_stream = st; }
     int e = 0;
diff --git a/lidar_snow_sim_amd/csrc/snowgpu_sort.hip b/lidar_snow_sim_amd/csrc/snowgpu_sort.hip
--- a/lidar_snow_sim_amd/csrc/snowgpu_sort.hip
+++ b/lidar_snow_sim_amd/csrc/snowgpu_sort.hip
@@ -88,9 +88,12 @@
 __global__ __launch_bounds__(SG_BLOCK) void k_sort_scan(const int64_t *__restrict__ frame_off,
                                                         const int32_t *__restrict__ tile_hist,
                                                         int32_t *__restrict__ tile_base, int64_t max_tiles,
-                                                        const int32_t *__restrict__ tile_unsorted, int32_t *__restrict__ frame_unsorted)
+                                                        const int32_t *__restrict__ tile_unsorted, int32_t *__restrict__ frame_unsorted, SgSortSeg sg)
 {
     const int f = blockIdx.x, v = threadIdx.x;
+    if (sg.tbl_cnt) {
+        for (int64_t i = (int64_t)f * SG_BLOCK + v; i < sg.n_zero; i += (int64_t)gridDim.x * SG_BLOCK) sg.zero[i] = 0ull;
+    }
     const int64_t n = frame_off[f + 1] - frame_off[f];
     const int64_t tiles = (n + SG_TILE - 1) / SG_TILE;
     const int32_t *h = tile_hist + (int64_t)f * max_tiles * 256;
@@ -110,6 +113,17 @@
         __syncthreads();
     }
     int run = s[v] - total;
+    if (sg.tbl_cnt) {
+        int key = sg.n_tables;
+        if (v < sg.n_las) {
+            const int64_t i = (int64_t)f * sg.n_las + v;
+            const int id = sg.table_ids[i];
+            SgTable d{};
+            if (id >= 0 && id < sg.n_tables) { d = sg.tables[id]; key = id; }
+            sg.resolved[i] = d;
+        }
+        if (total > 0) atomicAdd(&sg.tbl_cnt[(size_t)key * SG_TBL_STRIDE], (1ull << 32) | (unsigned long long)((total + sg.block - 1) / sg.block));
+    }
 #pragma unroll 8
     for (int64_t t = 0; t < tiles; ++t) { b[t * 256 + v] = run; run += h[t * 256 + v]; }
 }
@@ -118,59 +132,64 @@
 __global__ __launch_bounds__(SG_BLOCK) void k_sort_scatter(const T *__restrict__ rows, const uint8_t *__restrict__ ch8, const int64_t *__restrict__ frame_off,
                                                            const int32_t *__restrict__ tile_hist, const int32_t *__restrict__ tile_base,
                                                            const uint16_t *__restrict__ rank, int32_t *__restrict__ perm, T *__restrict__ srows,
-                                                           const int32_t *__restrict__ frame_unsorted, int identity_perm, int64_t max_tiles)
+                                                           const int32_t *__restrict__ frame_unsorted, int identity_perm, int64_t max_tiles, int per)
 {
     const int f = blockIdx.y;
     const int64_t base = frame_off[f], n = frame_off[f + 1] - base;
-    const int64_t tile0 = (int64_t)blockIdx.x * SG_TILE;
-    if (tile0 >= n) return;
+    const int64_t first_tile = (int64_t)blockIdx.x * per;
+    if (first_tile * SG_TILE >= n) return;
     const int tid = threadIdx.x;
     if (!frame_unsorted[f]) {
         if (identity_perm)
-            for (int q = 0; q < 4; ++q) { const int64_t r = tile0 + q * SG_BLOCK + tid; if (r < n) perm[base + r] = (int32_t)r; }
+            for (int64_t r = first_tile * SG_TILE + tid; r < n && r < (first_tile + per) * SG_TILE; r += SG_BLOCK) perm[base + r] = (int32_t)r;
         return;
     }
     __shared__ T stage[SG_TILE * 5];
     __shared__ int s_dest[SG_TILE];
     __shared__ uint16_t s_src[SG_TILE];
     __shared__ int s_start[256];
-    const int32_t *b = tile_base + ((int64_t)f * max_tiles + blockIdx.x) * 256;
-    {
-        const int c = tile_hist[((int64_t)f * max_tiles + blockIdx.x) * 256 + tid];
-        s_start[tid] = c;
+    for (int64_t tile = first_tile; tile < first_tile + per; ++tile) {
+        const int64_t tile0 = tile * SG_TILE;
+        if (tile0 >= n) break;
+        if (tile != first_tile) __syncthreads();
+        const int32_t *b = tile_base + ((int64_t)f * max_tiles + tile) * 256;
+        {
+            const int c = tile_hist[((int64_t)f * max_tiles + tile) * 256 + tid];
+            s_start[tid] = c;
+            __syncthreads();
+            for (int d = 1; d < 256; d <<= 1) {
+                const int add = tid >= d ? s_start[tid - d] : 0;
+                __syncthreads();
+                s_start[tid] += add;
+                __syncthreads();
+            }
+            const int excl = s_start[tid] - c;
+            __syncthreads();
+            s_start[tid] = excl;
+            __syncthreads();
+        }
+        const int m = (int)(n - tile0 < SG_TILE ? n - tile0 : SG_TILE);
+        for (int q = 0; q < 4; ++q) {
+            const int i = q * SG_BLOCK + tid;
+            if (i < m) {
+                const int64_t r = tile0 + i;
+                const int ch = ch8[base + r], rk = rank[base + r];
+                const int sp = s_start[ch] + rk;
+                const T *p = rows + (base + r) * 5;
+                const T v0 = p[0], v1 = p[1], v2 = p[2], v3 = p[3], v4 = p[4];
+                T *d = stage + sp * 5;
+                d[0] = v0; d[1] = v1; d[2] = v2; d[3] = v3; d[4] = v4;
+                s_dest[sp] = b[ch] + rk;
+                s_src[sp] = (uint16_t)i;
+            }
+        }
         __syncthreads();
-        for (int d = 1; d < 256; d <<= 1) {
-            const int add = tid >= d ? s_start[tid - d] : 0;
-            __syncthreads();
-            s_start[tid] += add;
-            __syncthreads();
-        }
-        const int excl = s_start[tid] - c;
-        __syncthreads();
-        s_start[tid] = excl;
-        __syncthreads();
-    }
-    const int m = (int)(n - tile0 < SG_TILE ? n - tile0 : SG_TILE);
-    for (int q = 0; q < 4; ++q) {
-        const int i = q * SG_BLOCK + tid;
-        if (i < m) {
-            const int64_t r = tile0 + i;
-            const int ch = ch8[base + r], rk = rank[base + r];
-            const int sp = s_start[ch] + rk;
-            const T *p = rows + (base + r) * 5;
-            const T v0 = p[0], v1 = p[1], v2 = p[2], v3 = p[3], v4 = p[4];
-            T *d = stage + sp * 5;
-            d[0] = v0; d[1] = v1; d[2] = v2; d[3] = v3; d[4] = v4;
-            s_dest[sp] = b[ch] + rk;
-            s_src[sp] = (uint16_t)i;
-        }
-    }
-    __syncthreads();
-    for (int idx = tid; idx < m * 5; idx += SG_BLOCK) {
-        const int sp = idx / 5, j = idx - sp * 5;
-        srows[(base + s_dest[sp]) * 5 + j] = stage[idx];
-    }
-    for (int sp = tid; sp < m; sp += SG_BLOCK) perm[base + s_dest[sp]] = (int32_t)(tile0 + s_src[sp]);
+        for (int idx = tid; idx < m * 5; idx += SG_BLOCK) {
+            const int sp = idx / 5, j = idx - sp * 5;
+            srows[(base + s_dest[sp]) * 5 + j] = stage[idx];
+        }
+        for (int sp = tid; sp < m; sp += SG_BLOCK) perm[base + s_dest[sp]] = (int32_t)(tile0 + s_src[sp]);
+    }
 }
 
 template <typename T>
@@ -209,29 +228,18 @@
     return r;
 }
 
-__global__ __launch_bounds__(256) void k_seg_count(const int64_t *__restrict__ frame_off, int n_frames, const int32_t *__restrict__ tile_base,
-                                                   int64_t max_tiles, const int32_t *__restrict__ table_ids, int n_las, int n_tables, int blk,
-                                                   unsigned long long *__restrict__ tbl_cnt, const SgTable *__restrict__ tables,
-                                                   SgTable *__restrict__ resolved)
-{
-    const int p = blockIdx.x * 256 + threadIdx.x;
-    if (p >= n_frames * 256) return;
-    if (resolved && (p & 255) < n_las) {
-        const int64_t i = (int64_t)(p >> 8) * n_las + (p & 255);
-        const int t = table_ids[i];
-        SgTable d{};
-        if (t >= 0 && t < n_tables) d = tables[t];
-        resolved[i] = d;
-    }
-    const SgPair r = sg_pair(p, frame_off, tile_base, max_tiles, table_ids, n_las, n_tables);
-    if (r.rows > 0) atomicAdd(&tbl_cnt[(size_t)r.key * SG_TBL_STRIDE], (1ull << 32) | (unsigned long long)((r.rows + blk - 1) / blk));
-}
-
 __global__ __launch_bounds__(1024) void k_seg_scan(unsigned long long *__restrict__ tbl_cnt, unsigned long long *__restrict__ tbl_base, int n,
-                                                   int32_t *__restrict__ seg_n, int32_t *__restrict__ one_chunk_blk)
+                                                   int32_t *__restrict__ seg_n, int32_t *__restrict__ one_chunk_blk, unsigned long long *__restrict__ tbl_cur,
+                                                   const int32_t *__restrict__ frame_unsorted, int n_frames, int32_t *__restrict__ hint_unsorted)
 {
     __shared__ unsigned long long sc[1024];
     const int t = threadIdx.x;
+    if (hint_unsorted) {
+        int u = 0;
+        for (int f = t; f < n_frames; f += 1024) u |= frame_unsorted[f];
+        u = __syncthreads_or(u);
+        if (t == 0) *hint_unsorted = u ? 1 : 0;
+    }
     const int per = (n + 1023) / 1024, b0 = t * per, b1 = b0 + per < n ? b0 + per : n;
     unsigned long long sum = 0;
     for (int k = b0; k < b1; ++k) sum += tbl_cnt[(size_t)k * SG_TBL_STRIDE];
@@ -239,7 +247,7 @@
     __syncthreads();
     for (int d = 1; d < 1024; d <<= 1) { const unsigned long long add = t >= d ? sc[t - d] : 0; __syncthreads(); sc[t] += add; __syncthreads(); }
     unsigned long long run = sc[t] - sum;
-    for (int k = b0; k < b1; ++k) { const unsigned long long c = tbl_cnt[(size_t)k * SG_TBL_STRIDE]; tbl_base[k] = run; run += c; tbl_cnt[(size_t)k * SG_TBL_STRIDE] = 0; }
+    for (int k = b0; k < b1; ++k) { const unsigned long long c = tbl_cnt[(size_t)k * SG_TBL_STRIDE]; tbl_base[k] = run; run += c; tbl_cnt[(size_t)k * SG_TBL_STRIDE] = 0; tbl_cur[(size_t)k * SG_TBL_STRIDE] = 0; }
     if (t == 1023) {
         seg_n[0] = (int32_t)(sc[1023] >> 32); seg_n[1] = (int32_t)(sc[1023] & 0xffffffffull);
         if (one_chunk_blk) { one_chunk_blk[0] = 0; one_chunk_blk[1] = (int32_t)(sc[1023] & 0xffffffffull); }
@@ -363,24 +371,28 @@
 extern "C" int sg_launch_sort(const void *rows, int dtype, const int64_t *frame_off, int n_frames, int64_t n_total,
                               int32_t *tile_hist, int32_t *tile_base, uint16_t *rank, uint8_t *ch8, int32_t *perm, int32_t *status,
                               int64_t max_tiles, const double *lean_plane, double *lean_part, int32_t *tile_unsorted, int32_t *frame_unsorted,
-                              void *srows, int identity_perm, int phase , void *stream)
+                              void *srows, int identity_perm, int phase , const SgSortSeg *seg, int scatter_tiles, void *stream)
 {
     (void)n_total;
     hipStream_t st = (hipStream_t)stream;
     dim3 grid((unsigned)max_tiles, (unsigned)n_frames);
     SgLeanTile lt{};
     lt.plane = lean_plane; lt.delta = 0.5; lt.part = lean_part; lt.max_tiles = max_tiles;
+    SgSortSeg sg{};
+    if (seg) sg = *seg;
+    const int per = (int)std::max<int64_t>(1, std::min<int64_t>(scatter_tiles, ((int64_t)n_frames * max_tiles) / 2048));
+    dim3 grid2((unsigned)((max_tiles + per - 1) / per), (unsigned)n_frames);
     return sg_by_dtype(dtype, [&](auto t) {
         using T = decltype(t);
         if (phase & 1) {
             if (lean_plane && lean_part) hipLaunchKernelGGL((k_sort_hist<T, true>), grid, dim3(SG_BLOCK), 0, st, (const T *)rows, frame_off, tile_hist, rank, ch8, status, max_tiles, lt, tile_unsorted);
             else hipLaunchKernelGGL((k_sort_hist<T, false>), grid, dim3(SG_BLOCK), 0, st, (const T *)rows, frame_off, tile_hist, rank, ch8, status, max_tiles, lt, tile_unsorted);
             SG_CHECK_LAUNCH();
-            hipLaunchKernelGGL(k_sort_scan, dim3(n_frames), dim3(SG_BLOCK), 0, st, frame_off, tile_hist, tile_base, max_tiles, tile_unsorted, frame_unsorted);
+            hipLaunchKernelGGL(k_sort_scan, dim3(n_frames), dim3(SG_BLOCK), 0, st, frame_off, tile_hist, tile_base, max_tiles, tile_unsorted, frame_unsorted, sg);
             SG_CHECK_LAUNCH();
         }
         if (phase & 2) {
-            hipLaunchKernelGGL(k_sort_scatter<T>, grid, dim3(SG_BLOCK), 0, st, (const T *)rows, ch8, frame_off, tile_hist, tile_base, rank, perm, (T *)srows, frame_unsorted, identity_perm, max_tiles);
+            hipLaunchKernelGGL(k_sort_scatter<T>, grid2, dim3(SG_BLOCK), 0, st, (const T *)rows, ch8, frame_off, tile_hist, tile_base, rank, perm, (T *)srows, frame_unsorted, identity_perm, max_tiles, per);
             SG_CHECK_LAUNCH();
         }
         return 0;
@@ -402,12 +414,17 @@
     });
 }
 
+extern "C" int sg_segments_small_fits(int n_frames, int n_tables, int64_t n_zero)
+{
+    return n_frames * 256 <= 1024 && n_tables + 1 <= SG_SEG_SMALL_TABLES && n_zero <= (1 << 16);
+}
+
 extern "C" int sg_launch_segments_small(const int64_t *frame_off, int n_frames, const int32_t *tile_base, int64_t max_tiles, const int32_t *table_ids,
                                         int n_las, int n_tables, int block, int32_t *seg_blk, int64_t *seg_start, int32_t *seg_cnt, int32_t *seg_frame,
                                         int32_t *seg_n, int32_t *seg_of_blk, int32_t *chunk_blk, const SgTable *tables, SgTable *resolved,
                                         unsigned long long *zero, int64_t n_zero, void *stream)
 {
-    if (n_frames * 256 > 1024 || n_tables + 1 > SG_SEG_SMALL_TABLES || n_zero > (1 << 16)) return -1;
+    if (!sg_segments_small_fits(n_frames, n_tables, n_zero)) return -1;
     hipLaunchKernelGGL(k_seg_small, dim3(1), dim3(1024), 0, (hipStream_t)stream, frame_off, n_frames, tile_base, max_tiles, table_ids, n_las, n_tables, block,
                        seg_start, seg_cnt, seg_frame, seg_blk, seg_of_blk, seg_n, chunk_blk, tables, resolved, zero, n_zero);
     SG_CHECK_LAUNCH();
@@ -415,20 +432,16 @@
 }
 
 extern "C" int sg_launch_segments(const int64_t *frame_off, int n_frames, const int32_t *tile_base, int64_t max_tiles, const int32_t *table_ids,
-                                  int n_las, int n_tables, int block, unsigned long long *tbl_cnt, unsigned long long *tbl_base, int32_t *seg_blk,
-                                  int64_t *seg_start, int32_t *seg_cnt, int32_t *seg_frame, int32_t *seg_n, int32_t *seg_of_blk,
-                                  int32_t *chunk_blk, const SgTable *tables, SgTable *resolved, void *stream)
+                                  int n_las, int n_tables, int block, unsigned long long *tbl_cnt, unsigned long long *tbl_cur, unsigned long long *tbl_base,
+                                  int32_t *seg_blk, int64_t *seg_start, int32_t *seg_cnt, int32_t *seg_frame, int32_t *seg_n, int32_t *seg_of_blk,
+                                  int32_t *chunk_blk, const int32_t *frame_unsorted, int32_t *hint_unsorted, void *stream)
 {
     hipStream_t st = (hipStream_t)stream;
     const unsigned grid = (unsigned)n_frames;
-    if (hipMemsetAsync(tbl_cnt, 0, sizeof(unsigned long long) * ((size_t)n_tables + 1) * SG_TBL_STRIDE, st) != hipSuccess) return (int)hipGetLastError();
-    hipLaunchKernelGGL(k_seg_count, dim3(grid), dim3(256), 0, st, frame_off, n_frames, tile_base, max_tiles, table_ids, n_las, n_tables, block, tbl_cnt,
-                       tables, resolved);
-    SG_CHECK_LAUNCH();
-    hipLaunchKernelGGL(k_seg_scan, dim3(1), dim3(1024), 0, st, tbl_cnt, tbl_base, n_tables + 1, seg_n, chunk_blk);
+    hipLaunchKernelGGL(k_seg_scan, dim3(1), dim3(1024), 0, st, tbl_cnt, tbl_base, n_tables + 1, seg_n, chunk_blk, tbl_cur, frame_unsorted, n_frames, hint_unsorted);
     SG_CHECK_LAUNCH();
     hipLaunchKernelGGL(k_seg_place, dim3(grid), dim3(256), 0, st, frame_off, n_frames, tile_base, max_tiles, table_ids, n_las, n_tables, block,
-                       tbl_base, tbl_cnt, seg_start, seg_cnt, seg_frame, seg_blk, seg_of_blk);
+                       tbl_base, tbl_cur, seg_start, seg_cnt, seg_frame, seg_blk, seg_of_blk);
     SG_CHECK_LAUNCH();
     return 0;
 }
```

New measurement: 10.54 billion, median of 6. About the same (+0.8%).
